# DavidLBick/espnet-1

Hardware: AMD Instinct MI355X
Metric: utterances/sec + step-time, Conformer-L T=1000 batch=32 @1/2/4/8 GPU (higher is better)
Workload: dtype bf16; 1 GPU; C3 Conformer-L (12x512, 8 heads, ff 2048, cnn 31) + 6-layer Transformer decoder, hybrid CTC/att 0.3/0.7, lsm 0.1, V=5000, T=1000 frames x 80, L=40, dropout 0.1, Adam+WarmupLR+clip 5; global_batch=32, seq_len=1000, parallelism=dp1

## Files before the change

espnet-1_amd/csrc/elementwise.hip:

```cpp
#include "common.h"

#include <cstdlib>
#include <cstring>

namespace {

__global__ void mvn_kernel(int B, int T, int F, const float* __restrict__ x, const long long* __restrict__ lens,
                           float* __restrict__ y) {
  const int b = blockIdx.x;
  const int f = threadIdx.x;
  __shared__ double red[1024];
  const long long L = lens[b];
  double s = 0.0;
  const int ty = threadIdx.y, ny = blockDim.y;
  if (f < F)
    for (int t = ty; t < T; t += ny)
      if (t < L) s += x[((long)b * T + t) * F + f];
  red[ty * blockDim.x + f] = s;
  __syncthreads();
  if (ty == 0 && f < F) {
    double a = 0.0;
    for (int k = 0; k < ny; ++k) a += red[k * blockDim.x + f];
    red[f] = a;
  }
// ... 1080 lines not shown
  if (dcol_dtype == EA_BF16 && dtype == EA_BF16) EA_C2I(bf16, bf16);
  else if (dcol_dtype == EA_BF16) EA_C2I(bf16, float);
  else if (dtype == EA_BF16) EA_C2I(float, bf16);
  else EA_C2I(float, float);
#undef EA_C2I
  EA_LAUNCH_CHECK();
  return 0;
}

extern "C" int ea_glu_fwd(long rows, int C, const void* x, int x_dtype, void* y, int y_dtype, void* stream) {
  EA_ENTRY();
  const long n = rows * C;
#define EA_G(TI, TO) hipLaunchKernelGGL((glu_fwd_kernel<TI, TO>), EA_GRID(n), rows, C, (const TI*)x, (TO*)y)
  if (x_dtype == EA_BF16 && y_dtype == EA_BF16) EA_G(bf16, bf16);
  else if (x_dtype == EA_BF16) EA_G(bf16, float);
  else if (y_dtype == EA_BF16) EA_G(float, bf16);
  else EA_G(float, float);
#undef EA_G
  EA_LAUNCH_CHECK();
  return 0;
}

extern "C" int ea_glu_bwd(long rows, int C, const void* x, int x_dtype, const float* dy, void* dx, void* stream) {
  EA_ENTRY();
  const long n = rows * C;
  if (x_dtype == EA_BF16)
    hipLaunchKernelGGL((glu_bwd_kernel<bf16, bf16>), EA_GRID(n), rows, C, (const bf16*)x, dy, (bf16*)dx);
  else
    hipLaunchKernelGGL((glu_bwd_kernel<float, float>), EA_GRID(n), rows, C, (const float*)x, dy, (float*)dx);
  EA_LAUNCH_CHECK();
  return 0;
}

extern "C" int ea_dwconv_fwd(int B, int T, int C, int K, const float* x, const float* w, const float* bias, float* y,
                             void* stream) {
  EA_ENTRY();
  EA_CHECK_ARG(K % 2 == 1);
  dim3 grid(B * ea_cdiv(T, DW_TT), ea_cdiv(C, DW_CT));
  dim3 gridr(B * ea_cdiv(T, 4 * DW_R), ea_cdiv(C, DW_CT));
  hipStream_t st = (hipStream_t)stream;
  switch (K) {
#define EA_DWF(KK) case KK: hipLaunchKernelGGL((dwconv_fwd_k_kernel<KK, DW_R>), gridr, dim3(256), 0, st, B, T, C, x, w, bias, y); break;
    EA_DWF(3) EA_DWF(5) EA_DWF(7) EA_DWF(15) EA_DWF(31)
#undef EA_DWF
    default: {
      const size_t sm = (size_t)(DW_TT + K - 1) * DW_CT * sizeof(float);
      hipLaunchKernelGGL(dwconv_fwd_kernel, grid, dim3(256), sm, st, B, T, C, K, x, w, bias, y);
    }
  }
  EA_LAUNCH_CHECK();
  return 0;
}

extern "C" int ea_dwconv_bwd(int B, int T, int C, int K, const float* x, const float* w, const float* dy, float* dx,
                             float* dw, float* dbias, int accumulate_params, float* workspace, long ws_elems,
                             void* stream) {
  EA_ENTRY();
  EA_CHECK_ARG(K % 2 == 1);
  const int nblk = B * ea_cdiv(T, DW_TT);
  dim3 grid(nblk, ea_cdiv(C, DW_CT));
  if (K == 3 || K == 5 || K == 7 || K == 15 || K == 31) {
    const int nblkr = B * ea_cdiv(T, 4 * DW_R);
    dim3 gridr(nblkr, ea_cdiv(C, DW_CT));
    const long rowlen = (long)C * (K + 1);
    EA_CHECK_ARG((long)nblkr * rowlen <= ws_elems);
    hipStream_t st = (hipStream_t)stream;
    switch (K) {
#define EA_DWB(KK) case KK: hipLaunchKernelGGL((dwconv_bwd_k_kernel<KK, DW_R>), gridr, dim3(256), 0, st, B, T, C, x, w, dy, dx, workspace); break;
      EA_DWB(3) EA_DWB(5) EA_DWB(7) EA_DWB(15) EA_DWB(31)
#undef EA_DWB
    }
    EA_LAUNCH_CHECK();
    int rc = ea_reduce_partials_tr(nblkr, C * K, workspace, rowlen, dw, accumulate_params, C, K, stream);
    if (rc || !dbias) return rc;
    return ea_reduce_partials(nblkr, C, workspace + (long)C * K, rowlen, dbias, accumulate_params, stream);
  }
  EA_CHECK_ARG((long)nblk * C * K <= ws_elems);
  const size_t sm = (size_t)(2 * (DW_TT + K - 1) + DW_TT) * DW_CT * sizeof(float);
  hipStream_t st = (hipStream_t)stream;
  hipLaunchKernelGGL(dwconv_bwd_kernel, grid, dim3(256), sm, st, B, T, C, K, x, w, dy, dx, workspace);
  EA_LAUNCH_CHECK();
  int rc = ea_reduce_partials(nblk, C * K, workspace, (long)C * K, dw, accumulate_params, stream);
  if (rc) return rc;
  if (dbias) return ea_colsum(B * T, C, dy, EA_F32, C, dbias, accumulate_params, workspace, ws_elems, stream);
  return 0;
}

extern "C" int ea_dwconv_fwd_glu(int B, int T, int C, int K, const void* g2, const float* w, const float* bias,
                                 float* y, void* stream) {
  EA_ENTRY();
  EA_CHECK_ARG((K == 3 || K == 5 || K == 7 || K == 15 || K == 31) && g2 && y && C % 4 == 0 &&
               ((uintptr_t)g2 % 8) == 0);
  dim3 gridr(B * ea_cdiv(T, 4 * DW_R), ea_cdiv(C, DW_CT));
  hipStream_t st = (hipStream_t)stream;
  switch (K) {
#define EA_DWF(KK)                                                                                          \
  case KK:                                                                                                  \
    hipLaunchKernelGGL((dwconv_fwd_k_kernel<KK, DW_R, true>), gridr, dim3(256), 0, st, B, T, C, (const float*)nullptr, \
                       w, bias, y, (const bf16*)g2);                                                        \
    break;
    EA_DWF(3) EA_DWF(5) EA_DWF(7) EA_DWF(15) EA_DWF(31)
#undef EA_DWF
  }
  EA_LAUNCH_CHECK();
  return 0;
}

extern "C" int ea_dwconv_fwd_glu_stats(int B, int T, int C, int K, const void* g2, const float* w, const float* bias,
                                       float* y, float* part, void* stream) {
  EA_ENTRY();
  EA_CHECK_ARG((K == 3 || K == 5 || K == 7 || K == 15 || K == 31) && g2 && y && part && bias && C % 4 == 0 &&
               ((uintptr_t)g2 % 8) == 0);
  dim3 gridr(B * ea_cdiv(T, 4 * DW_R), ea_cdiv(C, DW_CT));
  hipStream_t st = (hipStream_t)stream;
  switch (K) {
#define EA_DWF(KK)                                                                                            \
  case KK:                                                                                                    \
    hipLaunchKernelGGL((dwconv_fwd_k_kernel<KK, DW_R, true, true>), gridr, dim3(256), 0, st, B, T, C,           \
                       (const float*)nullptr, w, bias, y, (const bf16*)g2, part);                             \
    break;
    EA_DWF(3) EA_DWF(5) EA_DWF(7) EA_DWF(15) EA_DWF(31)
#undef EA_DWF
  }
  EA_LAUNCH_CHECK();
  return 0;
}

extern "C" int ea_dwconv_stats_parts(int B, int T, int* nparts) {
  EA_ENTRY();
  EA_CHECK_ARG(nparts != nullptr && B > 0 && T > 0);
  *nparts = B * ea_cdiv(T, 4 * DW_R);
  return 0;
}

extern "C" int ea_dwconv_glu_bwd(int B, int T, int C, int K, const float* x, const float* w, const float* dy,
                                 const void* g2, void* dg2, float* dw, float* dbias, int accumulate_params,
                                 float* workspace, long ws_elems, void* stream) {
  EA_ENTRY();
  EA_CHECK_ARG((K == 3 || K == 5 || K == 7 || K == 15 || K == 31) && g2 && dg2 && dw && dbias);
  EA_CHECK_ARG(x != nullptr || (C % 4 == 0 && ((uintptr_t)g2 % 8) == 0));
  const int nblkr = B * ea_cdiv(T, 4 * DW_R);
  dim3 gridr(nblkr, ea_cdiv(C, DW_CT));
  const long rowlen = (long)C * (K + 1);
  EA_CHECK_ARG((long)nblkr * rowlen <= ws_elems);
  hipStream_t st = (hipStream_t)stream;
  const bool adj = dbias == dw + (long)C * K;
  switch (K) {
#define EA_DWB(KK)                                                                                              \
  case KK:                                                                                                      \
    if (x)                                                                                                      \
      hipLaunchKernelGGL((dwconv_bwd_k_kernel<KK, DW_R, false, true>), gridr, dim3(256), 0, st, B, T, C, x, w, dy,   \
                         (float*)nullptr, workspace, (const bf16*)g2, (bf16*)dg2);                                    \
    else                                                                                                        \
      hipLaunchKernelGGL((dwconv_bwd_k_kernel<KK, DW_R, false, true, true>), gridr, dim3(256), 0, st, B, T, C,      \
                         (const float*)nullptr, w, dy, (float*)nullptr, workspace, (const bf16*)g2, (bf16*)dg2);      \
    break;
    EA_DWB(3) EA_DWB(5) EA_DWB(7) EA_DWB(15) EA_DWB(31)
#undef EA_DWB
  }
  EA_LAUNCH_CHECK();
  if (adj) return ea_reduce_partials_tr(nblkr, (int)rowlen, workspace, rowlen, dw, accumulate_params, C, K, stream);
  int rc = ea_reduce_partials_tr(nblkr, C * K, workspace, rowlen, dw, accumulate_params, C, K, stream);
  if (rc) return rc;
  return ea_reduce_partials(nblkr, C, workspace + (long)C * K, rowlen, dbias, accumulate_params, stream);
}


extern "C" int ea_add_pos_bias(long N, int H, int dk, const void* q, long ldq, const float* u, const float* v,
                               void* qu, void* qv, int dtype, void* stream) {
  EA_ENTRY();
  const long n = N * H * dk;
  if (dtype == EA_BF16)
    hipLaunchKernelGGL(add_pos_bias_kernel<bf16>, EA_GRID(n), N, H, dk, (const bf16*)q, ldq, u, v, (bf16*)qu, (bf16*)qv);
  else
    hipLaunchKernelGGL(add_pos_bias_kernel<float>, EA_GRID(n), N, H, dk, (const float*)q, ldq, u, v, (float*)qu, (float*)qv);
  EA_LAUNCH_CHECK();
  return 0;
}

extern "C" int ea_embed_fwd(long rows, int d, int L, const long long* tok, const float* E, float xscale,
                            const float* pe, float p, unsigned long long seed, float* y, void* stream) {
  EA_ENTRY();
  const long n = rows * d;
  hipLaunchKernelGGL(embed_fwd_kernel, EA_GRID(n), rows, d, L, tok, E, xscale, pe, p, (uint64_t)seed, ea_g_rng_salt, y);
  EA_LAUNCH_CHECK();
  return 0;
}

extern "C" int ea_add_pe_dropout(long rows, int d, int L, const float* pe, float p, unsigned long long seed,
                                 float* y, void* stream) {
  EA_ENTRY();
  EA_CHECK_ARG(rows >= 0 && d > 0 && L > 0);
  const long n = rows * d;
  if (n == 0) return 0;
  hipLaunchKernelGGL(add_pe_dropout_kernel, EA_GRID(n), n, d, L, pe, p, (uint64_t)seed, ea_g_rng_salt, y);
  EA_LAUNCH_CHECK();
  return 0;
}

extern "C" int ea_embed_bwd(long rows, int d, const long long* tok, const float* dy, float xscale, float p,
                            unsigned long long seed, float* dE, void* stream) {
  EA_ENTRY();
  EA_CHECK_ARG(rows >= 0 && rows <= EMBED_BWD_MAXROWS);
  if (rows == 0) return 0;
  hipLaunchKernelGGL(embed_bwd_kernel, dim3((unsigned)rows), dim3(256), 0, (hipStream_t)stream, (int)rows, d, tok,
                     dy, xscale, p, (uint64_t)seed, ea_g_rng_salt, dE);
  EA_LAUNCH_CHECK();
  return 0;
}

extern "C" int ea_argmax_rows(long rows, int V, const float* x, long ld, long long* out, void* stream) {
  EA_ENTRY();
  hipLaunchKernelGGL(argmax_rows_kernel, dim3(ea_cdiv(rows, 4)), dim3(256), 0, (hipStream_t)stream, rows, V, x, ld, out);
// ... 111 lines not shown
```

espnet-1_amd/csrc/gemm.hip:

```cpp

#include "gemm_kern.h"
#include <cstdio>
#include <cstdlib>

namespace {
__global__ void splitk_reduce(GemmP p) {
  const long MN = (long)p.M * p.N;
  const int z = blockIdx.y;
  const int zb = z / p.nh, zh = z % p.nh;
  const float* base = p.ws + (long)z * p.splitk * MN;
  const bool vec = p.vec_c && (p.N % 4 == 0);
  const EpiK ek = make_epik(p);
  const long n4 = vec ? MN / 4 : MN;
  for (long i = blockIdx.x * (long)blockDim.x + threadIdx.x; i < n4; i += (long)gridDim.x * blockDim.x) {
    if (vec) {
      float4 a = make_float4(0.f, 0.f, 0.f, 0.f);
      int s = 0;
      for (; s + 8 <= p.splitk; s += 8) {
        float4 b[8];
#pragma unroll
        for (int j = 0; j < 8; ++j) b[j] = *(const float4*)(base + (long)(s + j) * MN + i * 4);
#pragma unroll
        for (int j = 0; j < 8; ++j) { a.x += b[j].x; a.y += b[j].y; a.z += b[j].z; a.w += b[j].w; }
      }
      for (; s < p.splitk; ++s) {
        const float4 b = *(const float4*)(base + (long)s * MN + i * 4);
        a.x += b.x; a.y += b.y; a.z += b.z; a.w += b.w;
      }
      const int row = (int)(i * 4 / p.N), col = (int)(i * 4 % p.N);
      const float v[4] = {a.x, a.y, a.z, a.w};
      switch (p.epi.kind) {
        case EA_EPI_STORE: epi_four<EA_EPI_STORE>(p, ek, z, zb, zh, row, col, v); break;
        case EA_EPI_ACT: epi_four<EA_EPI_ACT>(p, ek, z, zb, zh, row, col, v); break;
        case EA_EPI_RESID: epi_four<EA_EPI_RESID>(p, ek, z, zb, zh, row, col, v); break;
        default: epi_four<EA_EPI_DACT>(p, ek, z, zb, zh, row, col, v); break;
      }
    } else {
      float a = 0.f;
      for (int s = 0; s < p.splitk; ++s) a += base[s * MN + i];
      epi_apply(p, z, zb, zh, (int)(i / p.N), (int)(i % p.N), a);
    }
  }
}

int g_gemm_stages = 2;
unsigned long long* g_probe = nullptr;
unsigned long long* g_diag = nullptr;
int g_gemm_bm64 = 1;
int g_gemm_bm32 = [] { const char* e = std::getenv("EA_GEMM_BM32"); return e ? std::atoi(e) : 1; }();
int g_gemm_pipe = 0;

int g_gemm_k128 = [] { const char* e = std::getenv("EA_GEMM_K128"); return e ? std::atoi(e) : 1; }();
int g_gemm_skinny = [] { const char* e = std::getenv("EA_GEMM_SKINNY"); return e ? std::atoi(e) : 16; }();

int launch_lds(GemmP& p, int a_k, int b_k, int nz, hipStream_t st, bool k128 = false) {
  dim3 grid(p.tiles_m * p.tiles_n, 1, nz * p.splitk);
  if (k128) return launch_k128(p, grid, st);
  if (p.g.mode != 0) {
    if (p.bm == 256 && g_gemm_pipe) return launch_pipe_conv(p, grid, st);
    return launch_lds_conv(p, grid, st);
  }
  if ((p.bm == 256 && p.bn == 256 && (g_gemm_pipe & 1)) ||
      (p.bm == 128 && p.bn == 128 && (g_gemm_pipe & 2)))
    return launch_pipe(p, a_k, b_k, grid, st);
  return launch_lds_dense(p, a_k, b_k, grid, st);
}

int g_force_bm = 0, g_force_bn = 0;
void choose_tile(GemmP& p, int a_k, long nz) {
  struct Cfg { int bm, bn, occ; double t0, rcu; bool ak_only; };
  static const Cfg cfgs[] = {{256, 256, 1, 12.4, 4.49, false}, {128, 128, 2, 8.3, 2.9, false},
                             {64, 128, 3, 6.8, 2.8, true}, {32, 128, 2, 6.0, 2.0, true}};
  p.bm = 128; p.bn = 128;
  if (g_force_bm) {
    if (g_force_bm <= 64 && !a_k) return;
    p.bm = g_force_bm; p.bn = g_force_bn;
    return;
  }
  double best = 1e300;
  for (const Cfg& c : cfgs) {
    if (c.ak_only && (!a_k || !g_gemm_bm64)) continue;
    if (c.bm == 32 && !g_gemm_bm32) continue;
    const long tiles = (long)ea_cdiv(p.M, c.bm) * ea_cdiv(p.N, c.bn) * nz;
    const double rounds = (double)((tiles + 256L * c.occ - 1) / (256L * c.occ));
    const double per_cu = (double)((tiles + 255) / 256) * 2.0 * c.bm * c.bn * (double)p.K * 1e-6;
    const double est = rounds * c.t0 + per_cu / c.rcu;
    if (est < best * 0.999) { best = est; p.bm = c.bm; p.bn = c.bn; }
  }
}

template <typename T>
int launch(GemmP& p, int a_k, int b_k, int nz, hipStream_t st, bool k128 = false) {
  if (sizeof(T) == 2 && p.lds) return launch_lds(p, a_k, b_k, nz, st, k128);
  if (p.bm != 128 || p.bn != 128) return EA_ERR_BAD_ARG;
  dim3 grid(p.tiles_m * p.tiles_n, 1, nz * p.splitk);
#define EA_GEMM_CASE(AKV, BKV)                                                      \
  if (a_k == AKV && b_k == BKV) {                                                   \
    hipLaunchKernelGGL((gemm_kernel<T, AKV, BKV>), grid, dim3(NT), 0, st, p);       \
  }
  EA_GEMM_CASE(true, true)
  else EA_GEMM_CASE(true, false)
  else EA_GEMM_CASE(false, true)
  else EA_GEMM_CASE(false, false)
#undef EA_GEMM_CASE
  EA_LAUNCH_CHECK();
  return 0;
}

}

extern "C" int ea_gemm_set_pipeline(int stages) {
  EA_ENTRY();
  EA_CHECK_ARG(stages == 0 || stages == 2 || stages == 12);
  g_gemm_bm64 = stages < 10;
  g_gemm_stages = stages % 10;
  return 0;
}

namespace {
__global__ void probe_begin_kernel(unsigned long long* s) { s[0] = ~0ull; s[1] = 0ull; }
__global__ void probe_end_kernel(unsigned long long* s) {
// ... 35 lines not shown
  EA_CHECK_ARG(state != nullptr && ring != nullptr && cap > 0 && phase >= 0 && phase <= 3 && opt != nullptr);
  hipLaunchKernelGGL(phase_stamp_kernel, dim3(1), dim3(1), 0, (hipStream_t)stream, state, ring, cap, phase,
                     &opt->next_lr, &opt->skip);
  EA_LAUNCH_CHECK();
  return 0;
}

extern "C" int ea_gemm_set_diag(unsigned long long* buf) {
  EA_ENTRY();
  g_diag = buf;
  return 0;
}

extern "C" int ea_gemm_set_probe(unsigned long long* slots) {
  EA_ENTRY();
  g_probe = slots;
  return 0;
}

extern "C" int ea_probe_begin(unsigned long long* slots, void* stream) {
  EA_ENTRY();
  EA_CHECK_ARG(slots != nullptr);
  hipLaunchKernelGGL(probe_begin_kernel, dim3(1), dim3(1), 0, (hipStream_t)stream, slots);
  EA_LAUNCH_CHECK();
  return 0;
}

extern "C" int ea_probe_end(unsigned long long* slots, void* stream) {
  EA_ENTRY();
  EA_CHECK_ARG(slots != nullptr);
  hipLaunchKernelGGL(probe_end_kernel, dim3(1), dim3(1), 0, (hipStream_t)stream, slots);
  EA_LAUNCH_CHECK();
  return 0;
}

extern "C" int ea_gemm_set_pipe(int on) {
  EA_ENTRY();
  g_gemm_pipe = on;
  return 0;
}

extern "C" int ea_gemm_set_k128(int mode, int slots) {
  EA_ENTRY();
  EA_CHECK_ARG(mode >= 0 && mode <= 3 && (slots == 3 || slots == 4));
  g_gemm_k128 = mode;
  eag::g_k128_slots = slots;
  return 0;
}

extern "C" int ea_gemm_set_skinny(int max_m) {
  EA_ENTRY();
  EA_CHECK_ARG(max_m >= 0 && max_m <= 64);
  g_gemm_skinny = max_m;
  return 0;
}

extern "C" int ea_gemm_set_tile(int bm, int bn) {
  EA_ENTRY();
  EA_CHECK_ARG((bm == 0 && bn == 0) || (bm == 32 && bn == 128) || (bm == 64 && bn == 128) ||
               (bm == 128 && bn == 128) || (bm == 256 && bn == 256));
  g_force_bm = bm;
  g_force_bn = bn;
  return 0;
}

static int gemm_impl(int dtype, int a_kmajor, int b_kmajor, int M, int N, int K,
                     const void* A, long lda, long sAb, long sAh,
                     const void* B, long ldb, long sBb, long sBh,
                     int batch, int nh,
                     void* C, int c_dtype, long ldc, long sCb, long sCh,
                     const ea_epilogue* epi, float* workspace, long ws_elems, void* stream,
                     const ea_conv_geo* geo, const float* w1x = nullptr, int w1T = 0, int w1F = 0,
                     float* w1part = nullptr, const uint8_t* w1pos = nullptr) {
  EA_CHECK_ARG(epi != nullptr && M >= 0 && N >= 0 && K >= 0 && batch >= 1 && nh >= 1);
  EA_CHECK_ARG(dtype == EA_F32 || dtype == EA_BF16);
  if (M == 0 || N == 0) return 0;
  const int E = dtype == EA_BF16 ? 8 : 4;
  const int esz = dtype == EA_BF16 ? 2 : 4;
  (void)esz;
  if (epi->kind == EA_EPI_RESID) EA_CHECK_ARG(c_dtype == EA_F32);
  GemmP p{};
  p.M = M; p.N = N; p.K = K;
  p.A = A; p.lda = lda; p.sAb = sAb; p.sAh = sAh;
  p.B = B; p.ldb = ldb; p.sBb = sBb; p.sBh = sBh;
  p.nh = nh;
  p.C = C; p.c_dtype = c_dtype; p.ldc = ldc; p.sCb = sCb; p.sCh = sCh;
  p.epi = *epi;
  p.ws = workspace;
  p.salt = ea_g_rng_salt;
  p.stamp = g_probe;
  p.diag = g_diag;
  p.g = geo ? *geo : ea_conv_geo{};
  p.w1x = w1x; p.w1part = w1part; p.w1pos = w1pos; p.w1T = w1T; p.w1F = w1F;
  p.vec_a = (lda % E == 0 && sAb % E == 0 && sAh % E == 0 && ((uintptr_t)A % 16) == 0);
  p.vec_b = (ldb % E == 0 && sBb % E == 0 && sBh % E == 0 && ((uintptr_t)B % 16) == 0);
  {
    const int ce = c_dtype == EA_BF16 ? 2 : 4;
    bool vc = (N % 4 == 0) && ldc % 4 == 0 && sCb % 4 == 0 && sCh % 4 == 0 && ((uintptr_t)C % (4 * ce)) == 0;
    if (epi->bias) vc = vc && ((uintptr_t)epi->bias % 16) == 0;
    if (epi->aux) vc = vc && epi->ldaux % 4 == 0 && ((uintptr_t)epi->aux % (4 * (epi->aux_dtype == EA_BF16 ? 2 : 4))) == 0;
    if (epi->resid) vc = vc && epi->ldr % 4 == 0 && ((uintptr_t)epi->resid % 16) == 0;
    p.vec_c = vc;
    bool v8 = vc && N % 8 == 0 && ldc % 8 == 0 && sCb % 8 == 0 && sCh % 8 == 0 && ((uintptr_t)C % 16) == 0;
    if (epi->aux) v8 = v8 && epi->ldaux % 8 == 0 && ((uintptr_t)epi->aux % 16) == 0;
    if (epi->resid) v8 = v8 && epi->ldr % 8 == 0;
    p.vec8 = v8;
  }
  p.bm = 128; p.bn = 128;
  if (dtype == EA_BF16 && M <= g_gemm_skinny && a_kmajor && b_kmajor && !geo && !w1part &&
      batch * nh == 1 && K % 32 == 0 && K > 0 && p.vec_a && p.vec_b) {
    static const bool trace_s = std::getenv("EA_GEMM_TRACE") != nullptr;
    if (trace_s) std::fprintf(stderr, "[ea_gemm] M=%d N=%d K=%d skinny epi=%d\n", M, N, K, (int)epi->kind);
    return launch_skinny(p, (hipStream_t)stream);
  }
  const double a_ext = 2.0 * ((a_kmajor ? (double)M : (double)K) * lda);
  const double b_ext = 2.0 * ((b_kmajor ? (double)N : (double)K) * ldb);
  const bool lds_path = dtype == EA_BF16 && p.vec_a && p.vec_b && g_gemm_stages > 0 &&
                        a_ext < 4.0e9 && b_ext < 4.0e9;
  p.lds = lds_path;
  if (geo && geo->mode != 0) {
    if (!lds_path || K % 64 != 0 || geo->C % 64 != 0 || batch * nh != 1) return EA_ERR_BAD_ARG;
    if ((geo->mode == EA_CONV_WGRAD) == (a_kmajor != 0) || (geo->mode == EA_CONV_FWD) != (b_kmajor != 0))
      return EA_ERR_BAD_ARG;
    choose_tile(p, 0, 1);
    if (geo->mode == EA_CONV_WGRAD && !g_force_bm) { p.bm = 256; p.bn = 256; }
    if (w1part) {
      if (!g_gemm_pipe || !p.vec8) return EA_ERR_BAD_ARG;
      p.bm = 256; p.bn = 256;
    }
    if (p.bm != 256 || p.bn != 256) { p.bm = 128; p.bn = 128; }
  } else if (lds_path) {
    choose_tile(p, a_kmajor, (long)batch * nh);
  }
  bool k128 = false;
  if (g_gemm_k128 && lds_path && !geo && a_kmajor && b_kmajor && K % 64 == 0 && K > 0) {
    const long t128 = (long)ea_cdiv(M, 128) * ea_cdiv(N, 128) * batch * nh;
    const bool fits = g_gemm_k128 == 3 ||
                      (!g_force_bm && (p.bm == 64 || p.bm == 128) && p.bn == 128 && t128 >= 128 &&
                       (g_gemm_k128 == 2 || (t128 <= 256 && K >= 1024)));
    if (fits) { p.bm = 128; p.bn = 128; k128 = true; }
  }
  if (p.bm <= 64 && !a_kmajor) return EA_ERR_BAD_ARG;
  p.tiles_m = ea_cdiv(M, p.bm);
  p.tiles_n = ea_cdiv(N, p.bn);
  const int KT = dtype == EA_BF16 ? KCfg<bf16>::KT : KCfg<float>::KT;
  const int nz = batch * nh;
  int splitk = 1;
  const long tiles = max(1L, (long)p.tiles_m * p.tiles_n * nz * (p.bm * p.bn) / (128 * 128));
  if (geo && geo->mode == EA_CONV_WGRAD && p.bm == 256) {
    if (workspace) {
      splitk = max(1, 256 / (p.tiles_m * p.tiles_n));
      splitk = min(splitk, K / (4 * KT));
      while (splitk > 1 && (long)splitk * M * N > ws_elems) --splitk;
      splitk = max(splitk, 1);
    }
  } else if (!k128 && workspace && tiles < 200 && K >= 16 * KT && K >= 1024 && (long)p.tiles_m * p.tiles_n * nz < 128) {
    splitk = (int)((384 + tiles - 1) / tiles);
    splitk = min(splitk, K / (4 * KT));
    splitk = min(splitk, 16);
    while (splitk > 1 && (long)splitk * nz * M * N > ws_elems) --splitk;
    if (splitk < 1) splitk = 1;
  }
  int kchunk = K;
  if (splitk > 1) {
    kchunk = ea_cdiv(ea_cdiv(K, splitk), KT) * KT;
    splitk = ea_cdiv(K, kchunk);
  }
  p.splitk = splitk;
  p.kchunk = kchunk;
  static const bool trace = std::getenv("EA_GEMM_TRACE") != nullptr;
  if (trace)
    std::fprintf(stderr, "[ea_gemm] M=%d N=%d K=%d ak=%d bk=%d nz=%d tile=%dx%d%s splitk=%d epi=%d geo=%d lds=%d\n", M,
                 N, K, a_kmajor, b_kmajor, nz, p.bm, p.bn, k128 ? "k" : "", splitk, (int)epi->kind, geo ? geo->mode : 0,
                 (int)p.lds);
  hipStream_t st = (hipStream_t)stream;
  int rc = dtype == EA_BF16 ? launch<bf16>(p, a_kmajor, b_kmajor, nz, st, k128)
                            : launch<float>(p, a_kmajor, b_kmajor, nz, st);
  if (rc) return rc;
  if (splitk > 1) {
    const long MN = (long)M * N;
    dim3 grid(ea_grid_cap(ea_cdiv(MN / 4 + 1, 256), 2048), nz);
    hipLaunchKernelGGL(splitk_reduce, grid, dim3(256), 0, st, p);
    EA_LAUNCH_CHECK();
  }
  return 0;
}

extern "C" int ea_gemm(int dtype, int a_kmajor, int b_kmajor, int M, int N, int K,
                       const void* A, long lda, long sAb, long sAh,
                       const void* B, long ldb, long sBb, long sBh,
                       int batch, int nh,
                       void* C, int c_dtype, long ldc, long sCb, long sCh,
                       const ea_epilogue* epi, float* workspace, long ws_elems, void* stream) {
  EA_ENTRY();
  return gemm_impl(dtype, a_kmajor, b_kmajor, M, N, K, A, lda, sAb, sAh, B, ldb, sBb, sBh, batch, nh, C, c_dtype,
                   ldc, sCb, sCh, epi, workspace, ws_elems, stream, nullptr);
}

extern "C" int ea_gemm_ln(int M, int N, int K, const float* x, long ldx, const float* gamma, const float* beta,
                          float eps, const void* W, long ldw, void* C, int c_dtype, long ldc, const ea_epilogue* epi,
                          void* stream) {
  EA_ENTRY();
  EA_CHECK_ARG(epi != nullptr && M >= 0 && N >= 0 && K > 0 && K % 32 == 0 && K <= 32 * 8 * 8);
  EA_CHECK_ARG(x && gamma && beta && W && C && ldx >= K && ldw >= K && ldc >= N);
  EA_CHECK_ARG(ldx % 4 == 0 && ((uintptr_t)x % 16) == 0 && ldw % 8 == 0 && ((uintptr_t)W % 16) == 0 &&
               ((uintptr_t)gamma % 16) == 0 && ((uintptr_t)beta % 16) == 0);
  if (epi->kind == EA_EPI_RESID) EA_CHECK_ARG(c_dtype == EA_F32);
  if (M == 0 || N == 0) return 0;
  GemmP p{};
  p.M = M; p.N = N; p.K = K;
  p.A = x; p.lda = ldx;
  p.B = W; p.ldb = ldw;
  p.nh = 1; p.splitk = 1; p.kchunk = K;
  p.C = C; p.c_dtype = c_dtype; p.ldc = ldc;
  p.epi = *epi;
  p.salt = ea_g_rng_salt;
  const int ce = c_dtype == EA_BF16 ? 2 : 4;
  bool vc = (N % 4 == 0) && ldc % 4 == 0 && ((uintptr_t)C % (4 * ce)) == 0;
  if (epi->bias) vc = vc && ((uintptr_t)epi->bias % 16) == 0;
  if (epi->aux) vc = vc && epi->ldaux % 4 == 0 && ((uintptr_t)epi->aux % (4 * (epi->aux_dtype == EA_BF16 ? 2 : 4))) == 0;
  if (epi->resid) vc = vc && epi->ldr % 4 == 0 && ((uintptr_t)epi->resid % 16) == 0;
  p.vec_c = vc;
  return launch_skinny_ln(p, gamma, beta, eps, (hipStream_t)stream);
}

extern "C" int ea_gemm_conv(const ea_conv_geo* geo, int a_kmajor, int b_kmajor, int M, int N, int K,
                            const void* A, long lda, const void* B, long ldb, void* C, int c_dtype, long ldc,
                            const ea_epilogue* epi, float* workspace, long ws_elems, void* stream) {
  EA_ENTRY();
  EA_CHECK_ARG(geo != nullptr && geo->mode >= EA_CONV_FWD && geo->mode <= EA_CONV_WGRAD);
  return gemm_impl(EA_BF16, a_kmajor, b_kmajor, M, N, K, A, lda, 0, 0, B, ldb, 0, 0, 1, 1, C, c_dtype, ldc, 0, 0,
                   epi, workspace, ws_elems, stream, geo);
}

extern "C" int ea_gemm_conv_w1(const ea_conv_geo* geo, int M, int N, int K, const void* A, long lda, const void* B,
                               long ldb, const ea_epilogue* epi, const float* x, int T, int Fin, float* part,
                               void* stream) {
  EA_ENTRY();
  EA_CHECK_ARG(geo != nullptr && geo->mode == EA_CONV_DGRAD && x != nullptr && part != nullptr);
  EA_CHECK_ARG(epi != nullptr && epi->kind == EA_EPI_DACT && epi->act == EA_ACT_RELU && epi->aux != nullptr &&
               epi->aux_dtype == EA_BF16);
  EA_CHECK_ARG(T >= 3 && Fin >= 3 && M < (1 << 24));
  return gemm_impl(EA_BF16, 1, 0, M, N, K, A, lda, 0, 0, B, ldb, 0, 0, 1, 1, nullptr, EA_BF16, N, 0, 0, epi,
                   nullptr, 0, stream, geo, x, T, Fin, part);
}

extern "C" int ea_gemm_conv_w1b(const ea_conv_geo* geo, int M, int N, int K, const void* A, long lda, const void* B,
                                long ldb, const ea_epilogue* epi, const float* x, int T, int Fin, float* part,
                                const unsigned char* pos, void* stream) {
  EA_ENTRY();
  EA_CHECK_ARG(geo != nullptr && geo->mode == EA_CONV_DGRAD && x != nullptr && part != nullptr && pos != nullptr);
  EA_CHECK_ARG(epi != nullptr && epi->kind == EA_EPI_DACT && epi->act == EA_ACT_RELU && N % 8 == 0);
  EA_CHECK_ARG(T >= 3 && Fin >= 3 && M < (1 << 24));
  return gemm_impl(EA_BF16, 1, 0, M, N, K, A, lda, 0, 0, B, ldb, 0, 0, 1, 1, nullptr, EA_BF16, N, 0, 0, epi,
                   nullptr, 0, stream, geo, x, T, Fin, part, pos);
}


extern "C" int ea_gemm_conv_w1b_all(const ea_conv_geo* geo, int N, const void* A, long lda, const void* B, long ldb,
                                    const ea_epilogue* epi, const float* x, int T, int Fin, float* part,
                                    const unsigned char* pos, void* stream) {
  EA_ENTRY();
  EA_CHECK_ARG(geo != nullptr && geo->mode == EA_CONV_DGRAD && x != nullptr && part != nullptr && pos != nullptr);
  EA_CHECK_ARG(epi != nullptr && epi->kind == EA_EPI_DACT && epi->act == EA_ACT_RELU);
  EA_CHECK_ARG(N >= 8 && N % 8 == 0 && geo->C % 64 == 0 && T >= 3 && Fin >= 3 && g_gemm_pipe != 0);
  EA_CHECK_ARG(lda % 8 == 0 && ldb % 8 == 0 && ((uintptr_t)A % 16) == 0 && ((uintptr_t)B % 16) == 0);
  GemmP p{};
  p.N = N;
  p.A = A; p.lda = lda;
  p.B = B; p.ldb = ldb;
  p.nh = 1; p.splitk = 1;
  p.C = nullptr; p.c_dtype = EA_BF16; p.ldc = N;
  p.epi = *epi;
  p.salt = ea_g_rng_salt;
  p.stamp = g_probe;
  p.diag = g_diag;
  p.g = *geo;
  p.w1x = x; p.w1part = part; p.w1pos = pos; p.w1T = T; p.w1F = Fin;
  p.vec_a = p.vec_b = p.vec_c = p.vec8 = p.lds = 1;
  p.bm = p.bn = 256;
  p.tiles_n = ea_cdiv(N, 256);
  int items = 0, tiles = 0;
  for (int c = 0; c < 4; ++c) {
    const int a = c >> 1, e = c & 1;
    const long rows = (long)geo->B * geo->nI[a] * geo->nJ[e];
    EA_CHECK_ARG(rows < (1L << 24));
    if (rows == 0) continue;
    const int k = p.ncls++;
    p.cls_item0[k] = items;
    p.cls_M[k] = (int)rows;
    p.cls_K[k] = (a ? 1 : 2) * (e ? 1 : 2) * geo->C;
    p.cls_a[k] = a;
    p.cls_e[k] = e;
    p.cls_tile0[k] = tiles;
    p.cls_pos[k] = geo->plane[c] / geo->C * (N / 8);
    tiles += (int)ea_cdiv(rows, 256);
    items += (int)ea_cdiv(rows, 256) * p.tiles_n;
  }
  if (p.ncls == 0) return 0;
  p.cls_item0[p.ncls] = items;
  p.M = p.cls_M[0]; p.K = p.cls_K[0]; p.kchunk = p.K; p.tiles_m = ea_cdiv(p.M, 256);
  const int unit = 8 * p.tiles_n;
  const dim3 grid((unsigned)(ea_cdiv(items, unit) * unit));
  static const bool trace = std::getenv("EA_GEMM_TRACE") != nullptr;
  if (trace) std::fprintf(stderr, "[ea_gemm] conv dgrad x%d classes, %d tiles, grid %u\n", p.ncls, items, grid.x);
  return launch_pipe_conv(p, grid, (hipStream_t)stream);
}
```

espnet-1_amd/csrc/gemm_kern.h:

```cpp
#pragma once
#include "common.h"


namespace eag {

constexpr int BM = 128, BN = 128, NT = 256;
constexpr int TILE_BYTES = 16384;

template <typename T> struct KCfg;
template <> struct KCfg<bf16> { static constexpr int KT = 64, KS = 32, E = 8, NKS = 2; };
template <> struct KCfg<float> { static constexpr int KT = 32, KS = 4, E = 4, NKS = 8; };

struct GemmP {
  int M, N, K;
  const void* A; long lda, sAb, sAh;
  const void* B; long ldb, sBb, sBh;
  int nh, splitk, kchunk;
  void* C; int c_dtype; long ldc, sCb, sCh;
  ea_epilogue epi;
  float* ws;
  int tiles_m, tiles_n;
  int vec_a, vec_b;
  int vec_c;
  int vec8;
// ... 256 lines not shown
    if (has_o) {
#pragma unroll
      for (int c = 0; c < 4; ++c) v[c] += e.beta * o[c];
    }
    st4(p.C, cidx, p.c_dtype, v);
  } else if constexpr (KIND == EA_EPI_ACT) {
    if (e.aux) st4(e.aux, (long)row * e.ldaux + col, e.aux_dtype, v);
    act_fwd_n<4>(e.act, v);
    drop4k(k, didx, v);
    st4(p.C, cidx, p.c_dtype, v);
  } else if constexpr (KIND == EA_EPI_RESID) {
    drop4k(k, didx, v);
#pragma unroll
    for (int c = 0; c < 4; ++c) v[c] = (has_o ? o[c] : 0.f) + e.rscale * v[c];
    st4(p.C, cidx, EA_F32, v);
  } else {
    drop4k(k, didx, v);
    act_bwd_mul_n<4>(e.act, v, o);
    st4(p.C, cidx, p.c_dtype, v);
  }
}

EA_DEV void ld8(const void* p, long i, int dt, float (&v)[8]) {
  if (dt == EA_BF16) {
    const uint4 u = *(const uint4*)((const bf16*)p + i);
    const bf16* b = (const bf16*)&u;
#pragma unroll
    for (int c = 0; c < 8; ++c) v[c] = (float)b[c];
  } else {
    const float4 f0 = *(const float4*)((const float*)p + i), f1 = *(const float4*)((const float*)p + i + 4);
    v[0] = f0.x; v[1] = f0.y; v[2] = f0.z; v[3] = f0.w; v[4] = f1.x; v[5] = f1.y; v[6] = f1.z; v[7] = f1.w;
  }
}
EA_DEV void st8(void* p, long i, int dt, const float (&v)[8]) {
  if (dt == EA_BF16) {
    union { uint4 u; bf16 b[8]; } t;
#pragma unroll
    for (int c = 0; c < 8; ++c) t.b[c] = (bf16)v[c];
    *(uint4*)((bf16*)p + i) = t.u;
  } else {
    *(float4*)((float*)p + i) = make_float4(v[0], v[1], v[2], v[3]);
    *(float4*)((float*)p + i + 4) = make_float4(v[4], v[5], v[6], v[7]);
  }
}
EA_DEV void drop8k(const EpiK& k, uint64_t idx, float (&v)[8]) {
  if (!k.drop) return;
#pragma unroll
  for (int q = 0; q < 4; ++q) {
    const uint32_t h = ea_pair_hash(k.key, (idx >> 1) + q);
    v[2 * q] *= (h & 0xffffu) >= k.thr ? k.sc : 0.f;
    v[2 * q + 1] *= (h >> 16) >= k.thr ? k.sc : 0.f;
  }
}
template <int KIND>
EA_DEV void epi_eight_pre(const GemmP& p, const EpiK& k, int z, int zb, int zh, int row, int col,
                          const float (&acc)[8], const float (&bias)[8], bool has_o, const float (&o)[8]) {
  const ea_epilogue& e = p.epi;
  const long cidx = zb * p.sCb + zh * p.sCh + (long)row * p.ldc + col;
  const uint64_t didx = ((uint64_t)z * p.M + row) * (uint64_t)p.N + col;
  float v[8];
#pragma unroll
  for (int c = 0; c < 8; ++c) v[c] = e.alpha * acc[c] + (KIND != EA_EPI_DACT ? bias[c] : 0.f);
  if constexpr (KIND == EA_EPI_STORE) {
#pragma unroll
    for (int c = 0; c < 8; ++c) v[c] *= e.post_scale;
    drop8k(k, didx, v);
    if (has_o) {
#pragma unroll
      for (int c = 0; c < 8; ++c) v[c] += e.beta * o[c];
    }
    st8(p.C, cidx, p.c_dtype, v);
  } else if constexpr (KIND == EA_EPI_ACT) {
    if (e.aux) st8(e.aux, (long)row * e.ldaux + col, e.aux_dtype, v);
    act_fwd_n<8>(e.act, v);
    drop8k(k, didx, v);
    st8(p.C, cidx, p.c_dtype, v);
  } else if constexpr (KIND == EA_EPI_RESID) {
    drop8k(k, didx, v);
#pragma unroll
    for (int c = 0; c < 8; ++c) v[c] = (has_o ? o[c] : 0.f) + e.rscale * v[c];
    st8(p.C, cidx, EA_F32, v);
  } else {
    drop8k(k, didx, v);
    act_bwd_mul_n<8>(e.act, v, o);
    st8(p.C, cidx, p.c_dtype, v);
  }
}

template <int KIND>
EA_DEV void epi_four(const GemmP& p, const EpiK& k, int z, int zb, int zh, int row, int col, const float (&acc)[4]) {
  float bias[4] = {0.f, 0.f, 0.f, 0.f}, o[4];
  if (p.epi.bias) {
    const float4 bb = *(const float4*)(p.epi.bias + col);
    bias[0] = bb.x; bias[1] = bb.y; bias[2] = bb.z; bias[3] = bb.w;
  }
  const bool has_o = epi_src<KIND>(p, zb, zh, row, col, o);
  epi_four_pre<KIND>(p, k, z, zb, zh, row, col, acc, bias, has_o, o);
}

template <int KIND, int NB>
EA_DEV void epi_batch(const GemmP& p, const EpiK& k, int z, int zb, int zh, const int (&rows)[NB],
                      const int (&cols)[NB], const float (&v)[NB][4]) {
  float o[NB][4];
  bool has[NB];
#pragma unroll
  for (int i = 0; i < NB; ++i) {
    has[i] = false;
    if (rows[i] < p.M && cols[i] < p.N) has[i] = epi_src<KIND>(p, zb, zh, rows[i], cols[i], o[i]);
  }
#pragma unroll
  for (int i = 0; i < NB; ++i) {
    if (rows[i] >= p.M || cols[i] >= p.N) continue;
    float bias[4] = {0.f, 0.f, 0.f, 0.f};
    if (KIND != EA_EPI_DACT && p.epi.bias) {
      const float4 bb = *(const float4*)(p.epi.bias + cols[i]);
      bias[0] = bb.x; bias[1] = bb.y; bias[2] = bb.z; bias[3] = bb.w;
    }
    epi_four_pre<KIND>(p, k, z, zb, zh, rows[i], cols[i], v[i], bias, has[i], o[i]);
  }
}

constexpr int EPI_LDT = 68;

template <typename T, bool AK, bool BKM>
__global__ __launch_bounds__(NT, 2) void gemm_kernel(GemmP p) {
  constexpr int KT = KCfg<T>::KT, NKS = KCfg<T>::NKS;
  __shared__ __attribute__((aligned(16))) char smem[2][2][TILE_BYTES];

  const int nt = p.tiles_m * p.tiles_n;
  const int b = blockIdx.x;
  const int q = nt / 8, r = nt % 8, xcd = b % 8;
  const int t = (xcd < r ? xcd * (q + 1) : r * (q + 1) + (xcd - r) * q) + b / 8;
  const int GM = 8;
  const int grp = t / (GM * p.tiles_n);
  const int gm0 = grp * GM;
  const int gsz = min(GM, p.tiles_m - gm0);
  const int tm = gm0 + (t % (GM * p.tiles_n)) % gsz;
  const int tn = (t % (GM * p.tiles_n)) / gsz;
// ... 126 lines not shown
                        uint4 (&v)[ROWS * 8 / NTT]) {
  constexpr int NCH = ROWS * 8 / NTT;
#pragma unroll
  for (int i = 0; i < NCH; ++i) {
    const int c = threadIdx.x + NTT * i;
    int mn, k;
    if (KMAJ) { mn = mn0 + (c >> 3); k = k0 + (c & 7) * 8; }
    else      { const int cj = c & 1023; k = k0 + (cj >> 4); mn = mn0 + (c >> 10) * 128 + (cj & 15) * 8; }
    const bf16* pp = KMAJ ? base + (long)mn * ld + k : base + (long)k * ld + mn;
    union { uint4 u; bf16 e[8]; } t;
#pragma unroll
    for (int e = 0; e < 8; ++e) {
      const bool ok = KMAJ ? (mn < MN && k + e < K) : (k < K && mn + e < MN);
      t.e[e] = ok ? pp[e] : (bf16)0.f;
    }
    v[i] = t.u;
  }
}
template <bool KMAJ, int ROWS, int NTT>
EA_DEV void store_tile_r(char* lds, const uint4 (&v)[ROWS * 8 / NTT]) {
#pragma unroll
  for (int i = 0; i < ROWS * 8 / NTT; ++i) {
    const int c = threadIdx.x + NTT * i;
    *(uint4*)(lds + img_off<KMAJ>(c)) = v[i];
  }
}

template <bool KMAJ>
EA_DEV bf16x8 frag_img(const char* img, int r, int ks, int lane) {
  if (KMAJ) return frag_bf16<true>(img, r, ks, lane);
  return frag_bf16<false>(img + (r >> 7) * 16384, r & 127, ks, lane);
}

struct TileIdx { int tm, tn, z, sk; };
EA_DEV TileIdx tile_index(const GemmP& p) {
  const int nt = p.tiles_m * p.tiles_n;
  const int total = gridDim.x * gridDim.z;
  const int bid = blockIdx.x + gridDim.x * blockIdx.z;
  const int q = total / 8, r = total % 8, xcd = bid % 8;
  const int w = (xcd < r ? xcd * (q + 1) : r * (q + 1) + (xcd - r) * q) + bid / 8;
  const int zz = w / nt, t = w - zz * nt;
  const int GM = 8;
  const int grp = t / (GM * p.tiles_n);
  const int gm0 = grp * GM;
  const int gsz = min(GM, p.tiles_m - gm0);
  TileIdx ti;
  ti.tm = gm0 + (t % (GM * p.tiles_n)) % gsz;
  ti.tn = (t % (GM * p.tiles_n)) / gsz;
  ti.z = zz / p.splitk;
  ti.sk = zz % p.splitk;
  return ti;
}

template <int KIND, int MI, int NJ>
EA_DEV void epi_wave(const GemmP& p, const EpiK& k, char* smem, int z, int zb, int zh, int r0, int c0, int lane,
                     int w, const f32x4 (&acc)[MI][NJ], int sk = 0) {
  constexpr int RC = MI < 4 ? MI : 4;
  constexpr int NG = RC * 4;
  constexpr int HB = NG < 8 ? NG : 8;
  constexpr int NCH = (MI / RC) * (NJ / 4), NBC = NG / HB, NU = NCH * NBC;
  float* t = (float*)smem + w * (RC * 16) * EPI_LDT;
  const int rq = (lane >> 4) * 4, cc = lane & 15, lc = (lane & 15) * 4;
  float* slab = p.splitk > 1 ? p.ws + ((long)z * p.splitk + sk) * (long)p.M * p.N : nullptr;
  const bool reads = p.vec_c && !slab &&
                     (KIND == EA_EPI_DACT || (KIND == EA_EPI_RESID && p.epi.resid) ||
                      (KIND == EA_EPI_STORE && p.epi.beta != 0.f));
  const void* src = nullptr;
  long sld = 0, sbase = 0;
  int sdt = EA_F32;
  if constexpr (KIND == EA_EPI_STORE) {
    src = p.C; sld = p.ldc; sbase = zb * p.sCb + zh * p.sCh; sdt = p.c_dtype;
  } else if constexpr (KIND == EA_EPI_RESID) {
    src = p.epi.resid; sld = p.epi.ldr;
  } else if constexpr (KIND == EA_EPI_DACT) {
    src = p.epi.aux; sld = p.epi.ldaux; sdt = p.epi.aux_dtype;
  }
  auto ch_rb = [&](int ch) { return r0 + (ch / (NJ / 4)) * RC * 16; };
  auto ch_col = [&](int ch) { return c0 + (ch % (NJ / 4)) * 64 + lc; };
  auto load_unit = [&](int u, float (&o)[HB][4]) {
    if (!reads) return;
    const int ch = u / NBC, h0 = (u % NBC) * HB;
    const int rb = ch_rb(ch), cl = min(ch_col(ch), p.N - 4);
    if (sdt == EA_BF16) {
#pragma unroll
      for (int it = 0; it < HB; ++it)
        vld4((const bf16*)src + sbase + (long)min(rb + (h0 + it) * 4 + (lane >> 4), p.M - 1) * sld + cl, o[it]);
    } else {
#pragma unroll
      for (int it = 0; it < HB; ++it)
        vld4((const float*)src + sbase + (long)min(rb + (h0 + it) * 4 + (lane >> 4), p.M - 1) * sld + cl, o[it]);
    }
  };
  auto transpose = [&](int ch) {
    const int ri = ch / (NJ / 4), cj = ch % (NJ / 4);
    if (ch > 0) {
      __builtin_amdgcn_wave_barrier();
      asm volatile("" ::: "memory");
    }
#pragma unroll
    for (int i = 0; i < RC; ++i)
#pragma unroll
      for (int j = 0; j < 4; ++j)
#pragma unroll
        for (int rr = 0; rr < 4; ++rr)
          t[(i * 16 + rq + rr) * EPI_LDT + j * 16 + cc] = acc[ri * RC + i][cj * 4 + j][rr];
    __builtin_amdgcn_wave_barrier();
    asm volatile("" ::: "memory");
  };
  if (!p.vec_c) {
#pragma unroll
    for (int ch = 0; ch < NCH; ++ch) {
      transpose(ch);
      const int rb = ch_rb(ch), col = ch_col(ch);
#pragma unroll 1
      for (int it = 0; it < NG; ++it) {
        const int lr = it * 4 + (lane >> 4), row = rb + lr;
        if (row >= p.M) continue;
#pragma unroll 1
        for (int c = 0; c < 4; ++c) {
          if (col + c >= p.N) break;
          const float x = t[lr * EPI_LDT + lc + c];
          if (slab) slab[(long)row * p.N + col + c] = x;
          else epi_one<KIND>(p, z, zb, zh, row, col + c, x);
        }
      }
    }
    return;
  }
  if (p.vec8) {
    constexpr int NG8 = RC * 2;
    constexpr int HB8 = NG8 < 4 ? NG8 : 4;
    const int lc8 = (lane & 7) * 8, rl = lane >> 3;
#pragma unroll
    for (int ch = 0; ch < NCH; ++ch) {
      transpose(ch);
      const int rb = ch_rb(ch), col = c0 + (ch % (NJ / 4)) * 64 + lc8;
      float bias[8] = {0.f, 0.f, 0.f, 0.f, 0.f, 0.f, 0.f, 0.f};
      if (!slab && KIND != EA_EPI_DACT && p.epi.bias && col < p.N) {
        const float4 b0 = *(const float4*)(p.epi.bias + col), b1 = *(const float4*)(p.epi.bias + col + 4);
        bias[0] = b0.x; bias[1] = b0.y; bias[2] = b0.z; bias[3] = b0.w;
        bias[4] = b1.x; bias[5] = b1.y; bias[6] = b1.z; bias[7] = b1.w;
      }
#pragma unroll
      for (int h0 = 0; h0 < NG8; h0 += HB8) {
        float o[HB8][8];
        if (reads) {
          const int cl = min(col, p.N - 8);
          if (sdt == EA_BF16) {
#pragma unroll
            for (int it = 0; it < HB8; ++it)
              ld8(src, sbase + (long)min(rb + (h0 + it) * 8 + rl, p.M - 1) * sld + cl, EA_BF16, o[it]);
          } else {
#pragma unroll
            for (int it = 0; it < HB8; ++it)
              ld8(src, sbase + (long)min(rb + (h0 + it) * 8 + rl, p.M - 1) * sld + cl, EA_F32, o[it]);
          }
        }
#pragma unroll
        for (int it = 0; it < HB8; ++it) {
          const int lr = (h0 + it) * 8 + rl, row = rb + lr;
          const float4 f0 = *(const float4*)(t + lr * EPI_LDT + lc8), f1 = *(const float4*)(t + lr * EPI_LDT + lc8 + 4);
          if (row >= p.M || col >= p.N) continue;
          if (slab) {
            *(float4*)(slab + (long)row * p.N + col) = f0;
            *(float4*)(slab + (long)row * p.N + col + 4) = f1;
            continue;
          }
          const float v[8] = {f0.x, f0.y, f0.z, f0.w, f1.x, f1.y, f1.z, f1.w};
          epi_eight_pre<KIND>(p, k, z, zb, zh, row, col, v, bias, reads, o[it]);
        }
      }
    }
    return;
  }
#pragma unroll
  for (int u = 0; u < NU; ++u) {
    const int ch = u / NBC, h0 = (u % NBC) * HB;
    const int rb = ch_rb(ch), col = ch_col(ch);
    if (u % NBC == 0) transpose(ch);
    float ob[HB][4];
    load_unit(u, ob);
    float bias[4] = {0.f, 0.f, 0.f, 0.f};
    if (!slab && KIND != EA_EPI_DACT && p.epi.bias && col < p.N) {
      const float4 bb = *(const float4*)(p.epi.bias + col);
      bias[0] = bb.x; bias[1] = bb.y; bias[2] = bb.z; bias[3] = bb.w;
    }
#pragma unroll
    for (int it = 0; it < HB; ++it) {
      const int lr = (h0 + it) * 4 + (lane >> 4), row = rb + lr;
      const float4 f = *(const float4*)(t + lr * EPI_LDT + lc);
      if (row >= p.M || col >= p.N) continue;
      const float v[4] = {f.x, f.y, f.z, f.w};
      if (slab) *(float4*)(slab + (long)row * p.N + col) = f;
      else epi_four_pre<KIND>(p, k, z, zb, zh, row, col, v, bias, reads, ob[it]);
    }
  }
}

EA_DEV int fdiv(int n, int d) {
  int q = (int)((float)n * __builtin_amdgcn_rcpf((float)d));
  if (q * d > n) --q;
  if ((q + 1) * d <= n) ++q;
  return q;
}
EA_DEV long x1p_row(const ea_conv_geo& g, int b, int t2, int f2, int kh, int kw) {
  const int a = kh & 1, e = kw & 1;
  return g.plane[a * 2 + e] + (((long)b * g.nI[a] + t2 + (kh >> 1)) * g.nJ[e] + f2 + (kw >> 1)) * g.C;
}
EA_DEV void dgrad_tap2(int a, int e, int q, int& kh, int& kw) {
  const int nkw = e ? 1 : 2;
  const int qh = q / nkw, qw = q - qh * nkw;
  kh = a ? 1 : 2 * qh;
  kw = e ? 1 : 2 * qw;
}
EA_DEV void dgrad_tap(const ea_conv_geo& g, int q, int& kh, int& kw) {
  const int nkw = g.e ? 1 : 2;
  const int qh = q / nkw, qw = q - qh * nkw;
  kh = g.a ? 1 : 2 * qh;
  kw = g.e ? 1 : 2 * qw;
}

template <int BM_, int BN_, int WN, bool AK, bool BKM, int STAGES, int MODE = 0>
// ... 176 lines not shown
          acc[i][j] = __builtin_amdgcn_mfma_f32_16x16x32_bf16(fa0[i], fb0[j], acc[i][j], 0, 0, 0);
#pragma unroll
      for (int i = 0; i < MI; ++i)
#pragma unroll
        for (int j = 0; j < NJ; ++j)
          acc[i][j] = __builtin_amdgcn_mfma_f32_16x16x32_bf16(fa1[i], fb1[j], acc[i][j], 0, 0, 0);
    } else {
#pragma unroll
      for (int ks = 0; ks < 2; ++ks) {
        bf16x8 fb[NJ];
#pragma unroll
        for (int j = 0; j < NJ; ++j) fb[j] = frag_img<BKM>(lb, wn + j * 16, ks, lane);
#pragma unroll
        for (int i = 0; i < MI; ++i) {
          const bf16x8 fa = frag_img<AK>(la, wm + i * 16, ks, lane);
#pragma unroll
          for (int j = 0; j < NJ; ++j)
            acc[i][j] = __builtin_amdgcn_mfma_f32_16x16x32_bf16(fa, fb[j], acc[i][j], 0, 0, 0);
        }
      }
    }
  };

  const int npre = min(STAGES - 1, nfull);
  for (int kt = 0; kt < npre; ++kt) issue(kt, kt);
  for (int kt = 0; kt < nfull; ++kt) {
    const int after = min(STAGES - 2, nfull - 1 - kt);
    if (after >= 2) wait_vmcnt<2 * GPT>();
    else if (after == 1) wait_vmcnt<GPT>();
    else wait_vmcnt<0>();
    lds_barrier();
    if (kt + STAGES - 1 < nfull) issue(kt + STAGES - 1, (kt + STAGES - 1) % STAGES);
    compute(kt % STAGES);
  }
  if (tail) {
    uint4 ra[BM_ * 8 / NTT], rb[BN_ * 8 / NTT];
    const int k0 = kbeg + nfull * BK;
    load_tile_r<AK, BM_, NTT>(A, p.lda, m0, p.M, k0, kend, ra);
    load_tile_r<BKM, BN_, NTT>(B, p.ldb, n0, p.N, k0, kend, rb);
    __syncthreads();
    char* base = smem + (nfull % STAGES) * STAGE_BYTES;
    store_tile_r<AK, BM_, NTT>(base, ra);
    store_tile_r<BKM, BN_, NTT>(base + A_BYTES, rb);
    __syncthreads();
    compute(nfull % STAGES);
  }

  __syncthreads();
  const EpiK ek = make_epik(p);
  switch (p.splitk > 1 ? EA_EPI_STORE : p.epi.kind) {
    case EA_EPI_STORE: epi_wave<EA_EPI_STORE, MI, NJ>(p, ek, smem, z, zb, zh, m0 + wm, n0 + wn, lane, w, acc, sk); break;
    case EA_EPI_ACT: epi_wave<EA_EPI_ACT, MI, NJ>(p, ek, smem, z, zb, zh, m0 + wm, n0 + wn, lane, w, acc, sk); break;
    case EA_EPI_RESID: epi_wave<EA_EPI_RESID, MI, NJ>(p, ek, smem, z, zb, zh, m0 + wm, n0 + wn, lane, w, acc, sk); break;
    default: epi_wave<EA_EPI_DACT, MI, NJ>(p, ek, smem, z, zb, zh, m0 + wm, n0 + wn, lane, w, acc, sk); break;
  }
  probe_end(p);
}

template <int OFF>
EA_DEV bf16x8 ds_read_b128_at(uint32_t addr) {
  bf16x8 v;
  asm volatile("ds_read_b128 %0, %1 offset:%2" : "=v"(v) : "v"(addr), "i"(OFF) : "memory");
  return v;
}

template <int S>
__global__ __launch_bounds__(512, 1) void gemm_k128(GemmP p) {
  constexpr int BK = 64, NTT = 512, NW = 8, MI = 4, NJ = 4;
  constexpr int A_BYTES = 128 * BK * 2, B_BYTES = 128 * BK * 2, STAGE = A_BYTES + B_BYTES;
  constexpr int ACH = A_BYTES / (NTT * 16), BCH = B_BYTES / (NTT * 16), G = ACH + BCH;
  constexpr int EPI_BYTES = 4 * 4 * 16 * EPI_LDT * 4;
  constexpr int HAND = EPI_BYTES;
  constexpr int SMEM = S * STAGE > HAND + 65536 ? S * STAGE : HAND + 65536;
  static_assert(S >= 3 && S <= 4, "ring depth");
  __shared__ __attribute__((aligned(1024))) char smem[SMEM];
  probe_start(p);

  const TileIdx ti = tile_index(p);
  const int m0 = ti.tm * 128, n0 = ti.tn * 128;
  const int z = ti.z, sk = ti.sk;
  const int zb = z / p.nh, zh = z % p.nh;
  const bf16* A = (const bf16*)p.A + zb * p.sAb + zh * p.sAh;
  const bf16* B = (const bf16*)p.B + zb * p.sBb + zh * p.sBh;
  const int kbeg = sk * p.kchunk;
  const int kend = min(p.K, kbeg + p.kchunk);
  const int nt = max(0, (kend - kbeg) / BK);
  const int tid = threadIdx.x, lane = tid & 63;
  const int w = __builtin_amdgcn_readfirstlane(tid >> 6);
  const int g = w >> 2, q = w & 3;
  const int wm = (q >> 1) * 64, wn = (q & 1) * 64;

  const __amdgpu_buffer_rsrc_t ra = __builtin_amdgcn_make_buffer_rsrc(
      (void*)(A + kbeg), (short)0, 0x7fffffff, 0x00020000);
  const __amdgpu_buffer_rsrc_t rb = __builtin_amdgcn_make_buffer_rsrc(
      (void*)(B + kbeg), (short)0, 0x7fffffff, 0x00020000);
  auto src = [&](long ld, int mn0, int MN, int ci) -> uint32_t {
    const int row = ci >> 3, c = (ci & 7) ^ swz_k(ci >> 3);
    return (uint32_t)(((long)min(mn0 + row, MN - 1) * ld + c * 8) * 2);
  };
  uint32_t aoff[ACH], boff[BCH];
#pragma unroll
  for (int i = 0; i < ACH; ++i) aoff[i] = src(p.lda, m0, p.M, (i * NW + w) * 64 + lane);
#pragma unroll
  for (int i = 0; i < BCH; ++i) boff[i] = src(p.ldb, n0, p.N, (i * NW + w) * 64 + lane);

  auto issue = [&](int t) {
    char* base = smem + (t % S) * STAGE;
// ... 529 lines not shown
  for (int k = 1; k < 4; ++k) c += (k < p.ncls && item >= p.cls_item0[k]) ? 1 : 0;
  const int local = item - p.cls_item0[c];
  ov.M = p.cls_M[c];
  ov.a = p.cls_a[c];
  ov.e = p.cls_e[c];
  ov.w1part = p.w1part + (long)p.cls_tile0[c] * 10 * p.N;
  ov.w1pos = p.w1pos + p.cls_pos[c];
  ti.tm = local / tn_n;
  ti.tn = local % tn_n;
  ti.z = 0;
  ti.sk = p.cls_K[c];
  return true;
}

template <bool AK, bool BKM, int MODE, int BT, int NS>
EA_DEV void pipe_body(const GemmP& p, const TileOv& ov, const TileIdx& ti, char* smem) {
  using PC = PipeT<BT, NS>;
  constexpr int MI = PC::MI;
  const int tm = ti.tm, m0 = ti.tm * BT, n0 = ti.tn * BT;
  const bool cls = MODE == EA_CONV_DGRAD && p.ncls;
  const int z = ti.z, sk = cls ? 0 : ti.sk;
  const int zb = z / p.nh, zh = z % p.nh;
  const bf16* A = (const bf16*)p.A + zb * p.sAb + zh * p.sAh;
  const bf16* B = (const bf16*)p.B + zb * p.sBb + zh * p.sBh;
  const int kbeg = sk * p.kchunk;
  const int kend = cls ? ti.sk : min(p.K, kbeg + p.kchunk);
  const int tid = threadIdx.x, lane = tid & 63, w = tid >> 6;
  const int wm = PC::wm(w), wn = PC::wn(w);
  f32x4 acc[MI][4];
#pragma unroll
  for (int i = 0; i < MI; ++i)
#pragma unroll
    for (int j = 0; j < 4; ++j) acc[i][j] = (f32x4){0.f, 0.f, 0.f, 0.f};
  diag_stamp(p, 0);
  float w1x[5];
  if constexpr (MODE == EA_CONV_DGRAD) {
    if (p.w1part) w1_load_x(p, ov, m0, w1x);
  }
  pipe_tile<AK, BKM, MODE, BT, NS>(p, ov, smem, A, B, m0, n0, kbeg, kend, acc);
  diag_stamp(p, 1);
  if constexpr (MODE == EA_CONV_DGRAD) {
    if (p.w1part) {
      w1_stage_x(smem + PC::SMEM, w1x);
      __syncthreads();
      w1_epilogue(p, ov, smem, m0, n0, wm, wn, lane, w, tm, acc);
      return;
    }
  }
  const EpiK ek = make_epik(p);
  switch (p.splitk > 1 ? EA_EPI_STORE : p.epi.kind) {
    case EA_EPI_STORE: epi_wave<EA_EPI_STORE, MI, 4>(p, ek, smem, z, zb, zh, m0 + wm, n0 + wn, lane, w, acc, sk); break;
    case EA_EPI_ACT: epi_wave<EA_EPI_ACT, MI, 4>(p, ek, smem, z, zb, zh, m0 + wm, n0 + wn, lane, w, acc, sk); break;
    case EA_EPI_RESID: epi_wave<EA_EPI_RESID, MI, 4>(p, ek, smem, z, zb, zh, m0 + wm, n0 + wn, lane, w, acc, sk); break;
    default: epi_wave<EA_EPI_DACT, MI, 4>(p, ek, smem, z, zb, zh, m0 + wm, n0 + wn, lane, w, acc, sk); break;
  }
  if (p.diag) {
    __syncthreads();
    diag_stamp(p, 2);
  }
}

template <bool AK, bool BKM, int MODE = 0, int BT = 256, int NS = 4>
__global__ __launch_bounds__(512, (PipeT<BT, NS>::OCC)) void gemm_pipe(GemmP p) {
  using PC = PipeT<BT, NS>;
  __shared__ __attribute__((aligned(1024))) char smem[MODE == EA_CONV_DGRAD ? W1_SMEM : PC::SMEM];
  probe_start(p);
  TileOv ov = tile_ov(p);
  TileIdx ti;
  bool run = true;
  if (MODE == EA_CONV_DGRAD && p.ncls) run = dgrad_class_item(p, ov, ti);
  else ti = tile_index(p);
  if (run) pipe_body<AK, BKM, MODE, BT, NS>(p, ov, ti, smem);
  probe_end(p);
}

}
```

espnet-1_amd/csrc/reduce.hip:

```cpp
#include "common.h"

namespace {

struct ColsumProbD {
  const void* x;
  float* part;
  long ld;
  int rows, n, dtype, rpp, ncb, item0;
};

struct ReduceProbD {
  const float* part;
  float* out;
  long stride;
  int nparts, n, accumulate, item0;
};

constexpr int CHUNK = 40;
template <typename P>
struct Chunk {
  int first, n;
  P pr[CHUNK];
};
static_assert(sizeof(Chunk<ColsumProbD>) <= 4000 && sizeof(Chunk<ReduceProbD>) <= 4000, "kernel argument space");

template <typename P>
__global__ void table_upload(Chunk<P> c, P* table) {
  for (int i = threadIdx.x; i < c.n; i += blockDim.x) table[c.first + i] = c.pr[i];
}

template <typename P>
EA_DEV int find_prob(const P* table, int n, int t) {
  int lo = 0, hi = n - 1;
  while (lo < hi) {
    const int mid = (lo + hi + 1) >> 1;
    if (__builtin_amdgcn_readfirstlane(table[mid].item0) <= t) lo = mid;
    else hi = mid - 1;
  }
  return lo;
}

__global__ __launch_bounds__(256) void colsum_grouped_kernel(const ColsumProbD* __restrict__ table, int nprob) {
  __shared__ float red[4][256];
  const int pi = find_prob(table, nprob, blockIdx.x);
  const ColsumProbD q = table[pi];
  const int it = blockIdx.x - q.item0;
  const int rb = it / q.ncb, cb = it - rb * q.ncb;
  const int lane = threadIdx.x & 63, w = threadIdx.x >> 6;
  const int c = cb * 256 + lane * 4;
  const int r0 = rb * q.rpp, r1 = min(q.rows, r0 + q.rpp);
  float a[4] = {0.f, 0.f, 0.f, 0.f};
  if (c < q.n) {
    if (q.dtype == EA_BF16) {
      const bf16* x = (const bf16*)q.x;
      int r = r0 + w;
      for (; r + 12 < r1; r += 16) {
        float v[4][4];
#pragma unroll
        for (int j = 0; j < 4; ++j) vld4(x + (long)(r + 4 * j) * q.ld + c, v[j]);
#pragma unroll
        for (int j = 0; j < 4; ++j)
#pragma unroll
          for (int k = 0; k < 4; ++k) a[k] += v[j][k];
      }
      for (; r < r1; r += 4) {
        float v[4];
        vld4(x + (long)r * q.ld + c, v);
#pragma unroll
        for (int k = 0; k < 4; ++k) a[k] += v[k];
      }
    } else {
      const float* x = (const float*)q.x;
      int r = r0 + w;
      for (; r + 12 < r1; r += 16) {
        float v[4][4];
#pragma unroll
        for (int j = 0; j < 4; ++j) vld4(x + (long)(r + 4 * j) * q.ld + c, v[j]);
#pragma unroll
        for (int j = 0; j < 4; ++j)
#pragma unroll
          for (int k = 0; k < 4; ++k) a[k] += v[j][k];
      }
      for (; r < r1; r += 4) {
        float v[4];
        vld4(x + (long)r * q.ld + c, v);
#pragma unroll
        for (int k = 0; k < 4; ++k) a[k] += v[k];
      }
    }
  }
#pragma unroll
  for (int k = 0; k < 4; ++k) red[w][lane * 4 + k] = a[k];
  __syncthreads();
  const int cc = cb * 256 + threadIdx.x;
  const int t = threadIdx.x;
  if (cc < q.n) q.part[(long)rb * q.n + cc] = (red[0][t] + red[1][t]) + (red[2][t] + red[3][t]);
}

constexpr int RP_CW = 16, RP_PL = 16;
__global__ __launch_bounds__(256) void reduce_grouped_kernel(const ReduceProbD* __restrict__ table, int nprob) {
  __shared__ double red[RP_PL][RP_CW];
  const int pi = find_prob(table, nprob, blockIdx.x);
  const ReduceProbD q = table[pi];
  const int cx = threadIdx.x % RP_CW, py = threadIdx.x / RP_CW;
  const int c = (blockIdx.x - q.item0) * RP_CW + cx;
  double a = 0.0;
  if (c < q.n) {
    int p = py;
    for (; p + 7 * RP_PL < q.nparts; p += 8 * RP_PL) {
      float v[8];
#pragma unroll
      for (int j = 0; j < 8; ++j) v[j] = q.part[(long)(p + RP_PL * j) * q.stride + c];
#pragma unroll
      for (int j = 0; j < 8; ++j) a += v[j];
    }
    for (; p < q.nparts; p += RP_PL) a += q.part[(long)p * q.stride + c];
  }
  red[py][cx] = a;
  __syncthreads();
  if (py == 0 && c < q.n) {
    double t = 0.0;
#pragma unroll
    for (int l = 0; l < RP_PL; ++l) t += red[l][cx];
    q.out[c] = q.accumulate ? q.out[c] + (float)t : (float)t;
  }
}

template <typename P>
int upload(const P* probs, int n, P* table, hipStream_t st) {
  Chunk<P> c{};
  for (int i = 0; i < n; ++i) {
    c.pr[c.n++] = probs[i];
    if (c.n == CHUNK || i == n - 1) {
      hipLaunchKernelGGL((table_upload<P>), dim3(1), dim3(64), 0, st, c, table);
      EA_LAUNCH_CHECK();
      c.first += c.n;
      c.n = 0;
    }
  }
  return 0;
}

}

extern "C" int ea_colsum_grouped(int n, const ea_colsum_prob* probs, void* ws, long ws_bytes, void* stream) {
  EA_ENTRY();
  EA_CHECK_ARG(n >= 0 && (n == 0 || (probs && ws)));
  if (n == 0) return 0;
  EA_CHECK_ARG((long)n * (long)sizeof(ColsumProbD) <= ws_bytes && n <= 4096);
  ColsumProbD* host = (ColsumProbD*)malloc(sizeof(ColsumProbD) * n);
  if (!host) return EA_ERR_BAD_ARG;
  long items = 0;
  int rc = 0;
  for (int i = 0; i < n && !rc; ++i) {
    const ea_colsum_prob& e = probs[i];
    const bool ok = e.x && e.part && e.rows > 0 && e.n > 0 && e.n % 4 == 0 && e.ld % 4 == 0 && e.rpp > 0 &&
                    (e.dtype == EA_BF16 || e.dtype == EA_F32) &&
                    ((uintptr_t)e.x % (e.dtype == EA_BF16 ? 8 : 16)) == 0;
    if (!ok) { rc = EA_ERR_BAD_ARG; break; }
    ColsumProbD& d = host[i];
    d.x = e.x; d.part = e.part; d.ld = e.ld;
    d.rows = e.rows; d.n = e.n; d.dtype = e.dtype; d.rpp = e.rpp;
    d.ncb = ea_cdiv(e.n, 256);
    d.item0 = (int)items;
    items += (long)ea_cdiv(e.rows, e.rpp) * d.ncb;
  }
  if (!rc && items >= (1L << 30)) rc = EA_ERR_BAD_ARG;
  hipStream_t st = (hipStream_t)stream;
  if (!rc) rc = upload(host, n, (ColsumProbD*)ws, st);
  free(host);
  if (rc) return rc;
  hipLaunchKernelGGL(colsum_grouped_kernel, dim3((unsigned)items), dim3(256), 0, st, (const ColsumProbD*)ws, n);
  EA_LAUNCH_CHECK();
  return 0;
}

extern "C" int ea_reduce_grouped(int n, const ea_reduce_prob* probs, void* ws, long ws_bytes, void* stream) {
  EA_ENTRY();
  EA_CHECK_ARG(n >= 0 && (n == 0 || (probs && ws)));
  if (n == 0) return 0;
  EA_CHECK_ARG((long)n * (long)sizeof(ReduceProbD) <= ws_bytes && n <= 4096);
  ReduceProbD* host = (ReduceProbD*)malloc(sizeof(ReduceProbD) * n);
  if (!host) return EA_ERR_BAD_ARG;
  long items = 0;
  int rc = 0;
  for (int i = 0; i < n; ++i) {
    const ea_reduce_prob& e = probs[i];
    if (!(e.part && e.out && e.n > 0 && e.nparts >= 0 && e.stride >= e.n)) { rc = EA_ERR_BAD_ARG; break; }
    ReduceProbD& d = host[i];
    d.part = e.part; d.out = e.out; d.stride = e.stride;
    d.nparts = e.nparts; d.n = e.n; d.accumulate = e.accumulate;
    d.item0 = (int)items;
    items += ea_cdiv(e.n, RP_CW);
  }
  if (!rc && items >= (1L << 30)) rc = EA_ERR_BAD_ARG;
  hipStream_t st = (hipStream_t)stream;
  if (!rc) rc = upload(host, n, (ReduceProbD*)ws, st);
  free(host);
  if (rc) return rc;
  hipLaunchKernelGGL(reduce_grouped_kernel, dim3((unsigned)items), dim3(256), 0, st, (const ReduceProbD*)ws, n);
  EA_LAUNCH_CHECK();
  return 0;
}

extern "C" int ea_grouped_table_bytes(int n, long* colsum_bytes, long* reduce_bytes) {
  EA_CHECK_ARG(n >= 0 && colsum_bytes && reduce_bytes);
  *colsum_bytes = (long)n * (long)sizeof(ColsumProbD);
  *reduce_bytes = (long)n * (long)sizeof(ReduceProbD);
  return 0;
}
```

espnet-1_amd/espnet_amd/deferred.py:

```python
from __future__ import annotations

import contextlib
import ctypes
import os

import torch

from ._lib import ColsumProb, GroupGemm, ReduceProb, dt, lib
from .streams import WGRAD, on_side, scratch, stream

GRAD_READY = None

DEFER_WGRAD = os.environ.get("EA_DEFER_WGRAD", "1") != "0"
DEFER_BUDGET = int(float(os.environ.get("EA_DEFER_BUDGET_MB", "8192")) * 2 ** 20)


def _nbytes(t):
    return t.numel() * t.element_size()


class WgradQueue:

    def __init__(self):
        self.active = False
# ... 47 lines not shown
                t.record_stream(cur)
        arr = (GroupGemm * n)()
        ntiles = 0
        for i, (K, dy, x, dw, M, N, lda, ldb, ldc, beta, _, _) in enumerate(items):
            arr[i] = GroupGemm(dy.data_ptr(), x.data_ptr(), dw.data_ptr(), lda, ldb, ldc, M, N, K, beta)
            ntiles += ((M + 255) // 256) * ((N + 255) // 256)
        nbytes = ctypes.c_long(0)
        lib.ea_gemm_grouped_ws_bytes(n, ntiles, ctypes.addressof(nbytes))
        ws = scratch("ggemm", nbytes.value, items[0][1].device)
        lib.ea_gemm_grouped(0, 0, n, ctypes.addressof(arr), ws.data_ptr(), ws.numel(), stream())
        for post in posts:
            post()

    def tensors(self):
        return [t for it in self.items for t in (it[1], it[2])]


WGRAD_Q = WgradQueue()

DEFER_REDUCE = os.environ.get("EA_DEFER_REDUCE", "1") != "0"


class ReduceQueue:

    def __init__(self):
        self.active = False
        self.colsums = []
        self.reduces = []
        self.spans = []
        self.pending = 0

    def _account(self, t):
        self.pending += _nbytes(t)
        if self.pending > DEFER_BUDGET:
            self.flush()

    def _claim(self, out, n):
        lo = out.data_ptr()
        hi = lo + 4 * n
        if any(lo < h and l_ < hi for l_, h in self.spans):
            self.flush()
        self.spans.append((lo, hi))

    def add_colsum(self, x, rows, n, ld, out, accumulate) -> bool:
        if x.dtype not in (torch.bfloat16, torch.float32) or out.dtype != torch.float32 or not out.is_contiguous():
            return False
        if rows <= 0 or n % 4 or ld % 4 or x.data_ptr() % (8 if x.dtype == torch.bfloat16 else 16):
            return False
        self._claim(out, n)
        self.colsums.append((x, rows, n, ld, out, accumulate))
        self._account(x)
        return True

    def add_reduce(self, part, nparts, n, stride, out, accumulate=True):
        self._claim(out, n)
        self.reduces.append((part, nparts, n, stride, out, accumulate))
        self._account(part)

    def tensors(self):
        return [c[0] for c in self.colsums] + [r[0] for r in self.reduces]

    def flush(self):
        if not self.colsums and not self.reduces:
            return
        colsums, reduces = self.colsums, list(self.reduces)
        self.colsums, self.reduces, self.spans = [], [], []
        self.pending = 0
        cur = torch.cuda.current_stream()
        for t in [c[0] for c in colsums] + [r[0] for r in reduces]:
            t.record_stream(cur)
        dev = (colsums[0][0] if colsums else reduces[0][0]).device
        cb, rb = ctypes.c_long(0), ctypes.c_long(0)
        if colsums:
            rpps = [max(32, (c[1] + 127) // 128) for c in colsums]
            nrbs = [(c[1] + r - 1) // r for c, r in zip(colsums, rpps)]
            part = torch.empty(sum(nrb * c[2] for c, nrb in zip(colsums, nrbs)), dtype=torch.float32, device=dev)
            arr = (ColsumProb * len(colsums))()
            off = 0
            for i, ((x, rows, n, ld, out, acc), rpp, nrb) in enumerate(zip(colsums, rpps, nrbs)):
                arr[i] = ColsumProb(x.data_ptr(), part.data_ptr() + 4 * off, ld, rows, n, dt(x), rpp)
                reduces.append((part, nrb, n, n, out, acc, off))
                off += nrb * n
            lib.ea_grouped_table_bytes(len(colsums), ctypes.addressof(cb), ctypes.addressof(rb))
            ws = scratch("colsum", cb.value, dev)
            lib.ea_colsum_grouped(len(colsums), ctypes.addressof(arr), ws.data_ptr(), ws.numel(), stream())
        arr = (ReduceProb * len(reduces))()
        for i, r in enumerate(reduces):
            part, nparts, n, stride, out, acc = r[:6]
            off = r[6] if len(r) > 6 else 0
            arr[i] = ReduceProb(part.data_ptr() + 4 * off, out.data_ptr(), stride, nparts, n, int(acc))
        lib.ea_grouped_table_bytes(len(reduces), ctypes.addressof(cb), ctypes.addressof(rb))
        ws = scratch("reduce", rb.value, dev)
        lib.ea_reduce_grouped(len(reduces), ctypes.addressof(arr), ws.data_ptr(), ws.numel(), stream())


REDUCE_Q = ReduceQueue()


def wgrad(*tensors, after=None, launches=False):
    if not launches and WGRAD_Q.active and REDUCE_Q.active:
        return contextlib.nullcontext()
    return WGRAD(*tensors, after=after)


def fork_event():
    return None if GRAD_READY is not None else WGRAD.fork_point()


def join_wgrad():
    WGRAD.join()
    WGRAD_Q.side_events = []


def grad_ready(bound):
    if GRAD_READY is not None:
        GRAD_READY(bound.prefix)
        return
    join_wgrad()


def _side_flush_ok():
    return GRAD_READY is None and WGRAD.enabled and torch.cuda.is_available()


def flush_wgrad_side(after=None):
    if WGRAD_Q.active and WGRAD_Q.items and _side_flush_ok():
        with WGRAD(*WGRAD_Q.tensors(), after=after):
            WGRAD_Q.flush()


def flush_deferred():
    WGRAD_Q.flush()
    REDUCE_Q.flush()


def deferred_tensors():
    return WGRAD_Q.tensors() + REDUCE_Q.tensors()


class deferred_wgrad:

    def __enter__(self):
        self.prev = (WGRAD_Q.active, REDUCE_Q.active)
# ... 20 lines not shown
```

espnet-1_amd/espnet_amd/hip_ops.py:

```python
from __future__ import annotations

import ctypes
import os
import sys
import types
import weakref

import torch

from . import deferred, streams
from ._lib import ACT_NONE, EPI_STORE, Epilogue, HipError, dt, lib
from .deferred import (REDUCE_Q, WGRAD_Q, deferred_tensors, deferred_wgrad, flush_deferred,
                       flush_wgrad_side, fork_event, grad_ready, join_wgrad, wgrad)
from .streams import aux, join_aux, mark_aux_fork, on_side, scratch, stream, take_aux_fork

_MOVED = {**dict.fromkeys(("DEBUG_DELAY_NS", "DEBUG_SERIAL", "OVERLAP_CTC_BWD"), streams),
          **dict.fromkeys(("GRAD_READY", "DEFER_WGRAD", "DEFER_REDUCE", "DEFER_BUDGET"), deferred)}


class _Ops(types.ModuleType):
    def __getattr__(self, name):
        if name in _MOVED:
            return getattr(_MOVED[name], name)
        raise AttributeError(f"module {self.__name__!r} has no attribute {name!r}")

    def __setattr__(self, name, value):
        if name in _MOVED:
            setattr(_MOVED[name], name, value)
        else:
            super().__setattr__(name, value)


sys.modules[__name__].__class__ = _Ops


class KernelProbe:

    TICK_MS = 1e-5

    def __init__(self, names, device=None):
        self.names = set(names)
        dev = device or torch.device("cuda", torch.cuda.current_device())
        self.slots = {n: torch.zeros(4, dtype=torch.int64, device=dev) for n in names}
        self.active = True

    def begin(self, name):
        if self.active and name in self.names:
            s = self.slots[name].data_ptr()
            lib.ea_probe_begin(s, stream())
            lib.ea_gemm_set_probe(s)

    def end(self, name):
        if self.active and name in self.names:
            lib.ea_gemm_set_probe(None)
            lib.ea_probe_end(self.slots[name].data_ptr(), stream())

    def reset(self):
        for t in self.slots.values():
            t.zero_()

    def mean_ms(self, name):
        tot, cnt = (int(x) for x in self.slots[name][2:4].tolist())
        return (tot / cnt * self.TICK_MS if cnt else float("nan")), cnt

# ... 146 lines not shown
        self.frozen = False

    def _rebuild(self):
        probs, tiles = [], []
        for pi, ((off, R, C), dst) in enumerate(self.items.items()):
            probs.append((off, dst.data_ptr(), R | (C << 32)))
            tiles += [(pi, tr, tc, 0) for tr in range((R + 63) // 64) for tc in range((C + 63) // 64)]
        dev = self.shadow.device
        self.probs = torch.tensor(probs, dtype=torch.int64).to(dev)
        self.tiles = torch.tensor(tiles, dtype=torch.int32).to(dev)
        self.ntiles = len(tiles)

    def get(self, w):
        off = (w.data_ptr() - self.shadow.data_ptr()) // w.element_size()
        key = (off, int(w.shape[0]), int(w.shape[1]))
        wt = self.items.get(key)
        if wt is None:
            if self.frozen or torch.cuda.is_current_stream_capturing():
                return None
            wt = torch.empty(key[2], key[1], dtype=w.dtype, device=w.device)
            self.items[key] = wt
            self._rebuild()
            self.refresh()
        return wt

    def refresh(self):
        if torch.cuda.is_current_stream_capturing():
            self.frozen = True
        if self.ntiles:
            lib.ea_transpose_bf16_grouped(self.ntiles, self.tiles.data_ptr(), self.probs.data_ptr(),
                                          self.shadow.data_ptr(), stream())


def attach_transposed_shadow(shadow):
    if not WT_SHADOW or shadow is None or shadow.dtype != torch.bfloat16:
        return None
    ts = TransposedShadow(shadow)
    TSHADOWS[shadow.untyped_storage().data_ptr()] = weakref.ref(ts)
    return ts


def _transposed(w):
    if not TSHADOWS or w.dtype != torch.bfloat16 or w.dim() != 2 or w.shape[1] > WT_MAX_KIN:
        return None
    if w.stride(1) != 1 or w.stride(0) != w.shape[1] or w.shape[0] % 8 or w.shape[1] % 8:
        return None
    ref = TSHADOWS.get(w.untyped_storage().data_ptr())
    ts = None if ref is None else ref()
    if ts is None or ts.shadow.untyped_storage().data_ptr() != w.untyped_storage().data_ptr():
        return None
    return ts.get(w)


def linear_dx(dy, w, out, *, epi: Epilogue = None):
    M, N, lda = _rows(dy)
    K = w.shape[1]
    _, _, ldc = _rows(out)
    wt = _transposed(w)
    if wt is not None:
        return gemm(dy, wt, out, M=M, N=K, K=N, a_kmajor=1, b_kmajor=1, lda=lda, ldb=wt.stride(0),
                    ldc=ldc, epi=epi)
    return gemm(dy, w, out, M=M, N=K, K=N, a_kmajor=1, b_kmajor=0, lda=lda, ldb=w.stride(0),
                ldc=ldc, epi=epi)


def linear_dw(dy, x, dw, *, accumulate=False, post=None):
    R, N, lddy = _rows(dy)
    R2, K, ldx = _rows(x)
    if R != R2:
        raise HipError("row mismatch in linear_dw")
    beta = 1.0 if accumulate else 0.0
    if WGRAD_Q.active and WGRAD_Q.add(dy, x, dw, M=N, N=K, K=R, lda=lddy, ldb=ldx, ldc=dw.stride(0), beta=beta,
                                      post=post):
        return dw
    gemm(dy, x, dw, M=N, N=K, K=R, a_kmajor=0, b_kmajor=0, lda=lddy, ldb=ldx,
         ldc=dw.stride(0), epi=make_epi(beta=beta))
    if post is not None:
        post()
    return dw


def layernorm_fwd(x, gamma, beta, y, mean, rstd, eps=1e-12):
    rows, d, ldx = _rows(x)
    lib.ea_layernorm_fwd(rows, d, x.data_ptr(), ldx, gamma.data_ptr(), beta.data_ptr(), eps,
                         y.data_ptr(), dt(y), y.stride(-2) if y.dim() > 1 else d,
                         mean.data_ptr(), rstd.data_ptr(), stream())


def linear_ln(x, gamma, beta, w, out, *, epi=None, eps=1e-12):
    rows, K, ldx = _rows(x)
    N = w.shape[0]
    if epi is None:
        epi = make_epi()
    lib.ea_gemm_ln(rows, N, K, x.data_ptr(), ldx, gamma.data_ptr(), beta.data_ptr(), ctypes.c_float(eps),
                   w.data_ptr(), w.stride(0), out.data_ptr(), dt(out), out.stride(0), ctypes.byref(epi), stream())
    return out


def layernorm_bwd(dy, x, gamma, mean, rstd, dx, dgamma, dbeta, accumulate=True, drop=None):
    rows, d, ldx = _rows(x)
    _, _, lddy = _rows(dy)
    _, _, lddx = _rows(dx)
    if drop is not None:
        y, ysc, yp, yseed = drop[:4]
        ycol = drop[4] if len(drop) > 4 else None
        _, _, ldy = _rows(y)
        dargs = (y.data_ptr(), dt(y), ldy, float(ysc), float(yp), yseed & 0xFFFFFFFFFFFFFFFF,
                 0 if ycol is None else ycol.data_ptr())
    if REDUCE_Q.active and rows > 0 and dbeta.data_ptr() == dgamma.data_ptr() + 4 * d:
        vec8 = (d % 8 == 0 and d <= 1024 and lddy % 8 == 0 and ldx % 4 == 0 and lddx % 4 == 0
                and x.data_ptr() % 16 == 0 and dy.data_ptr() % 16 == 0 and dx.data_ptr() % 16 == 0
                and gamma.data_ptr() % 16 == 0)
        nparts_max = (rows + 15) // 16 if vec8 else max((rows + 15) // 16, 128)
        part = torch.empty(nparts_max * (3 if drop is not None else 2) * d, dtype=torch.float32, device=x.device)
        np_ = ctypes.c_int(0)
        if drop is not None:
            yparts = ctypes.c_int(0)
            lib.ea_layernorm_bwd_partials_drop(rows, d, dy.data_ptr(), dt(dy), lddy, x.data_ptr(), ldx,
                                               gamma.data_ptr(), mean.data_ptr(), rstd.data_ptr(), dx.data_ptr(),
                                               lddx, int(accumulate), part.data_ptr(), part.numel(),
                                               ctypes.addressof(np_), *dargs, ctypes.addressof(yparts), stream())
            if yparts.value:
                npv = np_.value
                REDUCE_Q.add_reduce(part[npv * 2 * d:], npv, d, d, ycol, accumulate=True)
        else:
            lib.ea_layernorm_bwd_partials(rows, d, dy.data_ptr(), dt(dy), lddy, x.data_ptr(), ldx, gamma.data_ptr(),
                                          mean.data_ptr(), rstd.data_ptr(), dx.data_ptr(), lddx, int(accumulate),
                                          part.data_ptr(), part.numel(), ctypes.addressof(np_), stream())
        REDUCE_Q.add_reduce(part, np_.value, 2 * d, 2 * d, dgamma, accumulate=True)
        return
    w, n = f32_ws(x.device, max(1 << 22, 1024 * d))
    if drop is not None:
        lib.ea_layernorm_bwd_drop(rows, d, dy.data_ptr(), dt(dy), lddy, x.data_ptr(), ldx, gamma.data_ptr(),
                                  mean.data_ptr(), rstd.data_ptr(), dx.data_ptr(), lddx, int(accumulate),
                                  dgamma.data_ptr(), dbeta.data_ptr(), 1, w, n, *dargs, stream())
        return
    lib.ea_layernorm_bwd(rows, d, dy.data_ptr(), dt(dy), lddy, x.data_ptr(), ldx, gamma.data_ptr(),
                         mean.data_ptr(), rstd.data_ptr(), dx.data_ptr(), lddx, int(accumulate),
                         dgamma.data_ptr(), dbeta.data_ptr(), 1, w, n, stream())


def reduce_rows(part, nparts, n, stride, out, accumulate=True):
    if REDUCE_Q.active:
        REDUCE_Q.add_reduce(part, nparts, n, stride, out, accumulate)
        return
    lib.ea_reduce_partials(nparts, n, part.data_ptr(), stride, out.data_ptr(), int(accumulate), stream())


def colsum(x, out, accumulate=True, defer=True):
    rows, n, ld = _rows(x)
    if defer and REDUCE_Q.active and REDUCE_Q.add_colsum(x, rows, n, ld, out, accumulate):
        return
    w, wn = f32_ws(x.device)
    lib.ea_colsum(rows, n, x.data_ptr(), dt(x), ld, out.data_ptr(), int(accumulate), w, wn, stream())


def batchnorm_fwd(y, gamma, beta, mean, rstd, run_mean, run_var, nbt, z, training, act,
                  eps=1e-5, momentum=0.1):
    rows, C, _ = _rows(y)
    w, wn = f32_ws(y.device, (min(rows // 16 + 1, 256) + 2) * 2 * C)
    lib.ea_batchnorm_fwd(rows, C, y.data_ptr(), gamma.data_ptr(), beta.data_ptr(), eps, momentum,
                         int(training), mean.data_ptr(), rstd.data_ptr(), ptr(run_mean), ptr(run_var),
                         ptr(nbt), act, z.data_ptr(), dt(z), w, wn, stream())


def batchnorm_bwd(dz, y, mean, rstd, gamma, beta, act, dy, dgamma, dbeta):
    rows, C, _ = _rows(y)
    w, wn = f32_ws(y.device, (min(rows // 16 + 1, 256) + 2) * 2 * C)
    lib.ea_batchnorm_bwd(rows, C, dz.data_ptr(), dt(dz), y.data_ptr(), mean.data_ptr(), rstd.data_ptr(),
                         gamma.data_ptr(), beta.data_ptr(), act, dy.data_ptr(), dgamma.data_ptr(),
                         dbeta.data_ptr(), 1, w, wn, stream())


def scale_dropout(x, y, scale=1.0, p=0.0, seed=0):
    rows, cols, ldx = _rows(x)
    _, _, ldy = _rows(y)
    lib.ea_scale_dropout(rows, cols, x.data_ptr(), dt(x), ldx, y.data_ptr(), dt(y), ldy,
                         float(scale), float(p), seed & 0xFFFFFFFFFFFFFFFF, stream())
    return y


def scale_dropout_colsum(x, y, out, scale=1.0, p=0.0, seed=0, accumulate=True):
    scale_dropout(x, y, scale=scale, p=p, seed=seed)
    with wgrad(y):
        colsum(y, out, accumulate=accumulate)
    return y


def cast(x, dtype):
    if x.dtype == dtype:
        return x
    y = torch.empty(x.shape, dtype=dtype, device=x.device)
    scale_dropout(x.reshape(-1, x.shape[-1]), y.view(-1, y.shape[-1]))
    return y


def permute3(src, dst, A, Bd, Cd, accumulate=False):
    lib.ea_permute3(A, Bd, Cd, src.data_ptr(), dt(src), dst.data_ptr(), dt(dst), int(accumulate), stream())
```

espnet-1_amd/espnet_amd/layers/conformer.py:

```python
from __future__ import annotations

import ctypes
import os

import torch
from torch import nn

from .common import (ACT_SWISH, EPI_ACT, EPI_DACT, EPI_RESID, EPI_STORE, F32, Bound, attn_bwd, attn_dmask, dbd_layout,
                     attn_fused_bwd, attn_fwd, empty, fused_attn_ok, lib, ln_bwd, ln_fwd, math, ops, rup,
                     site_seed, dv_buf, drop_arg, site_dv, REL_LATEST, REL_LEGACY)



FUSE_DW_GLU = os.environ.get("EA_FUSE_DW_GLU", "1") != "0"
GLU_IN_CONV = os.environ.get("EA_GLU_IN_CONV", "1") != "0"
BN_STATS_IN_CONV = os.environ.get("EA_BN_STATS_IN_CONV", "1") != "0"


def _glu_in_conv(K, g2, d):
    return (GLU_IN_CONV and FUSE_DW_GLU and K in (3, 5, 7, 15, 31)
            and g2.dtype == torch.bfloat16 and d % 4 == 0 and g2.data_ptr() % 8 == 0 and torch.cuda.is_available())

class PositionwiseFeedForward(nn.Module):

# ... 66 lines not shown
        self.conv_module = conv_module
        self.norm_ff = LayerNorm(size)
        self.norm_mha = LayerNorm(size)
        if feed_forward_macaron is not None:
            self.norm_ff_macaron = LayerNorm(size)
            self.ff_scale = 0.5
        else:
            self.ff_scale = 1.0
        self.norm_conv = LayerNorm(size)
        self.norm_final = LayerNorm(size)
        self.size = size
        self.dropout_rate = dropout_rate
        self.layer_idx = 0
        self._b = None

    def bind(self, arena, prefix, cd):
        self._b = Bound(arena, prefix, cd)

    @staticmethod
    def arena_groups(prefix):
        a = prefix + "self_attn."
        return [[a + "linear_q.weight", a + "linear_k.weight", a + "linear_v.weight"],
                [a + "linear_q.bias", a + "linear_k.bias", a + "linear_v.bias"]]

    def forward(self, x, pos_emb, olens, seed):
        return ConformerBlockFn.apply(x, pos_emb, olens, self, seed, self.training)


def _ffn_fwd(L, b, x_in, pre, ln_name, p, seed_in, seed_out):
    cd = b.cd
    N, d = x_in.shape
    Fh = L.feed_forward.w_1.out_features
    xn, mu, rs = ln_fwd(x_in, b, ln_name, cd)
    h = empty(N, Fh, dtype=cd, device=x_in.device)
    a = empty(N, Fh, dtype=cd, device=x_in.device)
    ops.linear(xn, b.w(pre + ".w_1.weight"), a,
               epi=ops.make_epi(EPI_ACT, bias=b.f(pre + ".w_1.bias"), act=ACT_SWISH, aux=h,
                                drop_p=p, seed=seed_in))
    x_out = empty(N, d, device=x_in.device)
    ops.linear(a, b.w(pre + ".w_2.weight"), x_out,
               epi=ops.make_epi(EPI_RESID, bias=b.f(pre + ".w_2.bias"), resid=x_in,
                                rscale=L.ff_scale, drop_p=p, seed=seed_out))
    return x_out, (xn, mu, rs, h, a)


def _ffn_bwd(L, b, dx, x_in, saved, pre, ln_name, p, seed_in, seed_out, dv_in=None, next_drop=None):
    cd = b.cd
    xn, mu, rs, h, a = saved
    N, d = dx.shape
    dv = site_dv(dx, dv_in, b.g(pre + ".w_2.bias"), L.ff_scale, p, seed_out, cd)
    with ops.wgrad(dv, a):
        ops.linear_dw(dv, a, b.g(pre + ".w_2.weight"), accumulate=True)
    dh = empty(*h.shape, dtype=cd, device=dx.device)
    ops.linear_dx(dv, b.w(pre + ".w_2.weight"), dh,
                  epi=ops.make_epi(EPI_DACT, act=ACT_SWISH, aux=h, drop_p=p, seed=seed_in))
    with ops.wgrad(dh, xn):
        ops.colsum(dh, b.g(pre + ".w_1.bias"))
        ops.linear_dw(dh, xn, b.g(pre + ".w_1.weight"), accumulate=True)
    dxn = empty(N, d, dtype=cd, device=dx.device)
    ops.linear_dx(dh, b.w(pre + ".w_1.weight"), dxn)
    ln_bwd(dxn, x_in, b, ln_name, mu, rs, dx, accumulate=True, drop=next_drop)


class ConformerBlockFn(torch.autograd.Function):
    @staticmethod
    def forward(ctx, x, pos, olens, L: EncoderLayer, seed, training):
        b = L._b
        cd = b.cd
        B, T, d = x.shape
        N = B * T
        dev = x.device
        H = L.self_attn.h
        dk = d // H
        P2 = 2 * T - 1
        p = L.dropout_rate if training else 0.0
        pa = L.self_attn.dropout_rate if training else 0.0
        li = L.layer_idx
        sd = lambda s: site_seed(seed, li, s)
        x0 = x.reshape(N, d)
        x1, s_ff1 = _ffn_fwd(L, b, x0, "feed_forward_macaron", "norm_ff_macaron", p, sd(1), sd(2))
        xn2, mu2, rs2 = ln_fwd(x1, b, "norm_mha", cd)
        A = "self_attn."
        qkv = empty(N, 3 * d, dtype=cd, device=dev)
        ops.linear(xn2, b.w(A + "linear_q.weight", A + "linear_k.weight", A + "linear_v.weight",
                            shape=(3 * d, d)), qkv,
                   epi=ops.make_epi(bias=b.f(A + "linear_q.bias", A + "linear_k.bias",
                                             A + "linear_v.bias", shape=(3 * d,))))
        mode = L.self_attn.rel_mode
        fused = fused_attn_ok(cd, dk, T, T)
        if mode == REL_LEGACY and fused:
            shift = dbd_layout(T)[0]
            pp_full = empty(shift + P2, d, dtype=cd, device=dev)
            pp_full[:shift].zero_()
            pp = pp_full[shift:]
        else:
            pp_full = None
            pp = empty(P2, d, dtype=cd, device=dev)
        if mode == REL_LEGACY:
            assert pos.shape[0] == T
            pT = empty(T, d, dtype=cd, device=dev)
            ops.linear(pos, b.w(A + "linear_pos.weight"), pT)
            lib.ea_legacy_pext(T, d, pT.data_ptr(), d, pp.data_ptr(), d, ops.dt(pp), ops.stream())
        else:
            ops.linear(pos, b.w(A + "linear_pos.weight"), pp)
        scale = 1.0 / math.sqrt(dk)
        if fused:
            O = empty(N, d, dtype=cd, device=dev)
            lse = empty(B * H * T, device=dev)
            dmask, ldm = attn_dmask(B * H * T, T, pa, dev)
            lib.ea_attn_fused_fwd2_mode(B, H, T, T, dk, qkv.data_ptr(), 3 * d, qkv[:, d:].data_ptr(), 3 * d,
# ... 58 lines not shown
                                       bn_mean.data_ptr(), bn_rstd.data_ptr(), ops.ptr(bn.running_mean),
                                       ops.ptr(bn.running_var), ops.ptr(bn.num_batches_tracked), ACT_SWISH,
                                       z.data_ptr(), ops.dt(z), ops.stream())
        else:
            ops.batchnorm_fwd(y, b.f(C + "norm.weight"), b.f(C + "norm.bias"), bn_mean, bn_rstd,
                              bn.running_mean, bn.running_var, bn.num_batches_tracked, z,
                              training, ACT_SWISH, eps=bn.eps, momentum=bn.momentum)
        x3 = empty(N, d, device=dev)
        ops.linear(z, b.w(C + "pointwise_conv2.weight", shape=(d, d)), x3,
                   epi=ops.make_epi(EPI_RESID, bias=b.f(C + "pointwise_conv2.bias"), resid=x2,
                                    drop_p=p, seed=sd(5)))
        x4, s_ff2 = _ffn_fwd(L, b, x3, "feed_forward", "norm_ff", p, sd(6), sd(7))
        out, mu5, rs5 = ln_fwd(x4, b, "norm_final", F32)
        ctx.L = L
        ctx.meta = (B, T, d, H, dk, p, pa, seed, scale, ldT, mode)
        ctx.save = (x0, x1, x2, x3, x4, s_ff1, (xn2, mu2, rs2, qkv, pp, O, s_core),
                    (xn3, mu3, rs3, g2, glu, y, z, bn_mean, bn_rstd), s_ff2, (mu5, rs5), pos, olens)
        return out.view(B, T, d)

    @staticmethod
    def backward(ctx, dout):
        L = ctx.L
        b = L._b
        cd = b.cd
        B, T, d, H, dk, p, pa, seed, scale, ldT, mode = ctx.meta
        (x0, x1, x2, x3, x4, s_ff1, s_att, s_conv, s_ff2, (mu5, rs5), pos, olens) = ctx.save
        ctx.save = None
        li = L.layer_idx
        sd = lambda s: site_seed(seed, li, s)
        N = B * T
        dev = dout.device
        P2 = 2 * T - 1
        dx = empty(N, d, device=dev)
        dv_ff2 = dv_buf(N, d, cd, dev)
        ln_bwd(dout.reshape(N, d).contiguous(), x4, b, "norm_final", mu5, rs5, dx, accumulate=False,
               drop=drop_arg(dv_ff2, L.ff_scale, p, sd(7), b.g("feed_forward.w_2.bias")))
        dv_conv = dv_buf(N, d, cd, dev)
        _ffn_bwd(L, b, dx, x3, s_ff2, "feed_forward", "norm_ff", p, sd(6), sd(7), dv_in=dv_ff2,
                 next_drop=drop_arg(dv_conv, 1.0, p, sd(5), b.g("conv_module.pointwise_conv2.bias")))
        C = "conv_module."
        K = L.conv_module.kernel_size
        xn3, mu3, rs3, g2, glu, y, z, bn_mean, bn_rstd = s_conv
        dv = site_dv(dx, dv_conv, b.g(C + "pointwise_conv2.bias"), 1.0, p, sd(5), cd)
        with ops.wgrad(dv, z):
            ops.linear_dw(dv, z, b.g(C + "pointwise_conv2.weight", shape=(d, d)), accumulate=True)
        dz = empty(N, d, dtype=cd, device=dev)
        ops.linear_dx(dv, b.w(C + "pointwise_conv2.weight", shape=(d, d)), dz)
        dy = empty(N, d, device=dev)
        ops.batchnorm_bwd(dz, y, bn_mean, bn_rstd, b.f(C + "norm.weight"), b.f(C + "norm.bias"),
                          ACT_SWISH, dy, b.g(C + "norm.weight"), b.g(C + "norm.bias"))
        dg2 = empty(N, 2 * d, dtype=cd, device=dev)
        fuse = FUSE_DW_GLU and K in (3, 5, 7, 15, 31) and g2.dtype == torch.bfloat16
        if fuse:
            w, wn = ops.f32_ws(dev, B * ((T + 31) // 32) * d * (K + 1) + 1024)
            lib.ea_dwconv_glu_bwd(B, T, d, K, ops.ptr(glu), b.f(C + "depthwise_conv.weight").data_ptr(),
                                  dy.data_ptr(), g2.data_ptr(), dg2.data_ptr(),
                                  b.g(C + "depthwise_conv.weight").data_ptr(),
                                  b.g(C + "depthwise_conv.bias").data_ptr(), 1, w, wn, ops.stream())
        else:
            if glu is None:
                glu = empty(N, d, device=dev)
                lib.ea_glu_fwd(N, d, g2.data_ptr(), ops.dt(g2), glu.data_ptr(), 0, ops.stream())
            dglu = empty(N, d, device=dev)
            w, wn = ops.f32_ws(dev, B * ((T + 31) // 32) * d * (K + 1) + 1024)
            lib.ea_dwconv_bwd(B, T, d, K, glu.data_ptr(), b.f(C + "depthwise_conv.weight").data_ptr(),
                              dy.data_ptr(), dglu.data_ptr(), b.g(C + "depthwise_conv.weight").data_ptr(),
                              b.g(C + "depthwise_conv.bias").data_ptr(), 1, w, wn, ops.stream())
            lib.ea_glu_bwd(N, d, g2.data_ptr(), ops.dt(g2), dglu.data_ptr(), dg2.data_ptr(), ops.stream())
        with ops.wgrad(dg2, xn3):
            ops.colsum(dg2, b.g(C + "pointwise_conv1.bias"))
            ops.linear_dw(dg2, xn3, b.g(C + "pointwise_conv1.weight", shape=(2 * d, d)), accumulate=True)
        dxn3 = empty(N, d, dtype=cd, device=dev)
        ops.linear_dx(dg2, b.w(C + "pointwise_conv1.weight", shape=(2 * d, d)), dxn3)
        dv_att = dv_buf(N, d, cd, dev)
        ln_bwd(dxn3, x2, b, "norm_conv", mu3, rs3, dx, accumulate=True,
               drop=drop_arg(dv_att, 1.0, p, sd(4), b.g("self_attn.linear_out.bias")))
        A = "self_attn."
        xn2, mu2, rs2, qkv, pp, O, s_core = s_att
        dv = site_dv(dx, dv_att, b.g(A + "linear_out.bias"), 1.0, p, sd(4), cd)
        with ops.wgrad(dv, O):
            ops.linear_dw(dv, O, b.g(A + "linear_out.weight"), accumulate=True)
        dO = empty(N, d, dtype=cd, device=dev)
        ops.linear_dx(dv, b.w(A + "linear_out.weight"), dO)
        dqkv = empty(N, 3 * d, dtype=cd, device=dev)
        ldbd, shift = rup(P2, 8), 0
        if s_core[0] == "fused":
            _, lse, dmask, ldm, pp_full = s_core
            legacy = mode == REL_LEGACY
            shift, ldbd = dbd_layout(T)
            dbd = empty(H * B * T * ldbd, dtype=cd, device=dev)
            qv = empty(N, d, dtype=cd, device=dev)
            nqb = (T + 63) // 64
            part = empty(2 * B * nqb * d, device=dev)
            attn_fused_bwd(B=B, H=H, T1=T, T2=T, q=qkv, ldq=3 * d, k=qkv[:, d:], ldk=3 * d, v=qkv[:, 2 * d:],
                           ldv=3 * d, bu=b.f(A + "pos_bias_u"), bv=b.f(A + "pos_bias_v"), pp=pp, ldp=d,
                           klen=olens, causal=False, scale=scale, p=pa, seed=sd(3), O=O, ldo=d, lse=lse, dO=dO,
                           lddo=d, dq=dqkv, lddq=3 * d, dk=dqkv[:, d:], lddk=3 * d, dv=dqkv[:, 2 * d:],
                           lddv=3 * d, dbd=dbd, ldbd=ldbd, part=part, ldpart=d, qv_out=qv, ldqv=d, dmask=dmask,
                           ldm=ldm, flags=2 if legacy else 1 | 2, rel_mode=mode)
            ops.reduce_rows(part[:B * nqb * d], B * nqb, d, d, b.g(A + "pos_bias_u", shape=(d,)))
            if legacy:
                raw = dbd
                dbd = empty(H * B * T * ldbd, dtype=cd, device=dev)
                lib.ea_attn_legacy_band(H * B, T, raw.data_ptr(), dbd.data_ptr(), ldbd, ops.stream())
                del raw
                dqv = empty(N, d, dtype=cd, device=dev)
                ops.gemm(dbd, pp_full, dqv, M=T, N=dk, K=shift + P2, a_kmajor=1, b_kmajor=0, lda=ldbd, ldb=d, ldc=d,
                         batch=B, nh=H, sA=(T * ldbd, B * T * ldbd), sB=(0, dk), sC=(T * d, dk), splitk=False)
                ops.colsum(dqv, b.g(A + "pos_bias_v", shape=(d,)))
                lib.ea_add_2d(N, d, dqv.data_ptr(), ops.dt(dqv), d, dqkv.data_ptr(), ops.dt(dqkv), 3 * d, 1.0,
                              ops.stream())
            else:
                ops.reduce_rows(part[B * nqb * d:], B * nqb, d, d, b.g(A + "pos_bias_v", shape=(d,)))
        else:
            _, qu, qv, P, Pd = s_core
            dbd = empty(H * B * T * ldbd, dtype=cd, device=dev)
            attn_bwd(dO, qu, qkv[:, d:], qkv[:, 2 * d:], P, Pd, ldT, B=B, H=H, T1=T, T2=T, dk=dk,
                     ldq=d, ldk=3 * d, ldv=3 * d, scale=scale, p=pa, seed=sd(3), cd=cd,
                     dq=dqkv, lddq=3 * d, dk_=dqkv[:, d:], lddk=3 * d, dv=dqkv[:, 2 * d:], lddv=3 * d,
                     dbd=dbd, ldbd=ldbd, rel_mode=mode)
# ... 41 lines not shown
```

espnet-1_amd/espnet_amd/layers/decoder.py:

```python
from __future__ import annotations

import math

import torch
from torch import nn

from .common import (ACT_RELU, EPI_ACT, EPI_DACT, EPI_RESID, EPI_STORE, F32, Bound, attn_bwd,
                     attn_dmask, attn_fused_bwd, attn_fwd, empty, fused_attn_ok, lib, ln_bwd, ln_fwd, ops,
                     site_seed, dv_buf, drop_arg, site_dv)


def _mha_fwd(q, k, v, *, B, H, T1, T2, dk, ldq, ldk, ldv, klen, causal, scale, p, seed, cd):
    if fused_attn_ok(cd, dk, T1, T2):
        O = empty(B * T1, H * dk, dtype=cd, device=q.device)
        lse = empty(B * H * T1, device=q.device)
        dmask, ldm = attn_dmask(B * H * T1, T2, p, q.device)
        lib.ea_attn_fused_fwd2(B, H, T1, T2, dk, q.data_ptr(), ldq, k.data_ptr(), ldk, v.data_ptr(), ldv,
                               None, None, None, 0, klen.data_ptr(), int(causal), scale, float(p), seed,
                               O.data_ptr(), H * dk, lse.data_ptr(), ops.ptr(dmask), ldm, ops.stream())
        return O, ("fused", O, lse, dmask, ldm)
    O, P, Pd, ldT = attn_fwd(q, k, v, B=B, H=H, T1=T1, T2=T2, dk=dk, ldq=ldq, ldk=ldk, ldv=ldv, klen=klen,
                             causal=causal, scale=scale, p=p, seed=seed, cd=cd)
    return O, ("unfused", P, Pd, ldT)

# ... 147 lines not shown
                       epi=ops.make_epi(EPI_ACT, bias=b.f(ff + "w_1.bias"), act=ACT_RELU, aux=h,
                                        drop_p=p, seed=sd(l, 5)))
            x3 = empty(N, d, device=dev)
            ops.linear(a, b.w(ff + "w_2.weight"), x3,
                       epi=ops.make_epi(EPI_RESID, bias=b.f(ff + "w_2.bias"), resid=x2,
                                        drop_p=p, seed=sd(l, 6)))
            saved.append((x, x1, x2, (xn1, mu1, rs1, qkv, O1, st1),
                          (xn2, mu2, rs2, q2, O2, st2), (xn3, mu3, rs3, h, a)))
            x = x3
        xf, muf, rsf = ln_fwd(x, b, "after_norm", cd)
        logits = empty(N, V, device=dev)
        ops.linear(xf, b.w("output_layer.weight"), logits,
                   epi=ops.make_epi(bias=b.f("output_layer.bias")))
        ctx.dec = dec
        ctx.meta = (B, Tm, L, d, H, dk, nb, p, p_sa, p_src, p_pos, seed, scale)
        ctx.save = (mem, kv, ys_in, saved, x, xf, muf, rsf, hlens, ys_in_lens)
        return logits.view(B, L, V)

    @staticmethod
    def backward(ctx, dlogits):
        dec = ctx.dec
        b = dec._b
        cd = b.cd
        B, Tm, L, d, H, dk, nb, p, p_sa, p_src, p_pos, seed, scale = ctx.meta
        mem, kv, ys_in, saved, xlast, xf, muf, rsf, hlens, ys_in_lens = ctx.save
        ctx.save = None
        sd = lambda l, s: site_seed(seed, 100 + l, s)
        N, Nm = B * L, B * Tm
        V = dlogits.shape[-1]
        dev = dlogits.device
        dlog = ops.cast(dlogits.reshape(N, V).contiguous(), cd)
        with ops.wgrad(dlog, xf):
            ops.colsum(dlog, b.g("output_layer.bias"))
            ops.linear_dw(dlog, xf, b.g("output_layer.weight"), accumulate=True)
        dxf = empty(N, d, dtype=cd, device=dev)
        ops.linear_dx(dlog, b.w("output_layer.weight"), dxf)
        dx = empty(N, d, device=dev)
        dv_ff = dv_buf(N, d, cd, dev) if nb > 0 else None
        ln_bwd(dxf, xlast, b, "after_norm", muf, rsf, dx, accumulate=False,
               drop=None if dv_ff is None else
               drop_arg(dv_ff, 1.0, p, sd(nb - 1, 6), b.g(f"decoders.{nb - 1}.feed_forward.w_2.bias")))
        ldkv = 2 * d * nb
        dkv = empty(Nm, ldkv, dtype=cd, device=dev)
        for l in reversed(range(nb)):
            n = f"decoders.{l}."
            sa, xa, ff = n + "self_attn.", n + "src_attn.", n + "feed_forward."
            x0, x1, x2, s1, s2, s3 = saved[l]
            xn3, mu3, rs3, h, a = s3
            dv = site_dv(dx, dv_ff, b.g(ff + "w_2.bias"), 1.0, p, sd(l, 6), cd)
            with ops.wgrad(dv, a):
                ops.linear_dw(dv, a, b.g(ff + "w_2.weight"), accumulate=True)
            fork = ops.fork_event() if l < nb - 1 else None
            dh = empty(*h.shape, dtype=cd, device=dev)
            ops.linear_dx(dv, b.w(ff + "w_2.weight"), dh,
                          epi=ops.make_epi(EPI_DACT, act=ACT_RELU, aux=h, drop_p=p, seed=sd(l, 5)))
            if fork is not None:
                ops.flush_wgrad_side(after=fork)
            with ops.wgrad(dh, xn3):
                ops.colsum(dh, b.g(ff + "w_1.bias"))
                ops.linear_dw(dh, xn3, b.g(ff + "w_1.weight"), accumulate=True)
            dxn = empty(N, d, dtype=cd, device=dev)
            ops.linear_dx(dh, b.w(ff + "w_1.weight"), dxn)
            dv_src = dv_buf(N, d, cd, dev)
            ln_bwd(dxn, x2, b, n + "norm3", mu3, rs3, dx, accumulate=True,
                   drop=drop_arg(dv_src, 1.0, p, sd(l, 4), b.g(xa + "linear_out.bias")))
            xn2, mu2, rs2, q2, O2, st2 = s2
            dv = site_dv(dx, dv_src, b.g(xa + "linear_out.bias"), 1.0, p, sd(l, 4), cd)
            with ops.wgrad(dv, O2):
                ops.linear_dw(dv, O2, b.g(xa + "linear_out.weight"), accumulate=True)
            dO = empty(N, d, dtype=cd, device=dev)
            ops.linear_dx(dv, b.w(xa + "linear_out.weight"), dO)
            dq = empty(N, d, dtype=cd, device=dev)
            _mha_bwd(st2, dO, q2, kv[:, 2 * d * l:], kv[:, 2 * d * l + d:], B=B, H=H, T1=L, T2=Tm, dk=dk,
                     ldq=d, ldk=ldkv, ldv=ldkv, klen=hlens, causal=False, scale=scale, p=p_src,
                     seed=sd(l, 3), cd=cd, dq=dq, lddq=d, dk_=dkv[:, 2 * d * l:], lddk=ldkv,
                     dv=dkv[:, 2 * d * l + d:], lddv=ldkv)
            with ops.wgrad(dq, xn2):
                ops.colsum(dq, b.g(xa + "linear_q.bias"))
                ops.linear_dw(dq, xn2, b.g(xa + "linear_q.weight"), accumulate=True)
            dxn = empty(N, d, dtype=cd, device=dev)
            ops.linear_dx(dq, b.w(xa + "linear_q.weight"), dxn)
            dv_self = dv_buf(N, d, cd, dev)
            ln_bwd(dxn, x1, b, n + "norm2", mu2, rs2, dx, accumulate=True,
                   drop=drop_arg(dv_self, 1.0, p, sd(l, 2), b.g(sa + "linear_out.bias")))
            xn1, mu1, rs1, qkv, O1, st1 = s1
            dv = site_dv(dx, dv_self, b.g(sa + "linear_out.bias"), 1.0, p, sd(l, 2), cd)
            with ops.wgrad(dv, O1):
                ops.linear_dw(dv, O1, b.g(sa + "linear_out.weight"), accumulate=True)
            dO = empty(N, d, dtype=cd, device=dev)
            ops.linear_dx(dv, b.w(sa + "linear_out.weight"), dO)
            dqkv = empty(N, 3 * d, dtype=cd, device=dev)
            _mha_bwd(st1, dO, qkv, qkv[:, d:], qkv[:, 2 * d:], B=B, H=H, T1=L, T2=L, dk=dk,
                     ldq=3 * d, ldk=3 * d, ldv=3 * d, klen=ys_in_lens, causal=True, scale=scale, p=p_sa,
                     seed=sd(l, 1), cd=cd, dq=dqkv, lddq=3 * d, dk_=dqkv[:, d:], lddk=3 * d,
                     dv=dqkv[:, 2 * d:], lddv=3 * d)
            wn = (sa + "linear_q.weight", sa + "linear_k.weight", sa + "linear_v.weight")
            bn = (sa + "linear_q.bias", sa + "linear_k.bias", sa + "linear_v.bias")
            with ops.wgrad(dqkv, xn1):
                ops.colsum(dqkv, b.g(*bn, shape=(3 * d,)))
                ops.linear_dw(dqkv, xn1, b.g(*wn, shape=(3 * d, d)), accumulate=True)
            dxn = empty(N, d, dtype=cd, device=dev)
            ops.linear_dx(dqkv, b.w(*wn, shape=(3 * d, d)), dxn)
            dv_ff = dv_buf(N, d, cd, dev) if l > 0 else None
            ln_bwd(dxn, x0, b, n + "norm1", mu1, rs1, dx, accumulate=True,
                   drop=None if dv_ff is None else
                   drop_arg(dv_ff, 1.0, p, sd(l - 1, 6), b.g(f"decoders.{l - 1}.feed_forward.w_2.bias")))
        pe = dec.embed[1]
        lib.ea_embed_bwd(N, d, ys_in.data_ptr(), dx.data_ptr(), pe.xscale, p_pos, sd(0, 0),
                         b.g("embed.0.weight").data_ptr(), ops.stream())
        kvw, kvb = _kv_names(nb)
        with ops.wgrad(dkv, mem):
            ops.colsum(dkv, b.g(*kvb, shape=(ldkv,)))
# ... 6 lines not shown
```

espnet-1_amd/espnet_amd/layers/subsampling.py:

```python
from __future__ import annotations

import ctypes
import math
import os

import torch
from torch import nn

from .._lib import CONV_DGRAD, CONV_FWD, CONV_WGRAD, GEMM_PIPE, ConvGeo
from .common import (ACT_RELU, EPI_ACT, EPI_DACT, EPI_STORE, F32, Bound, empty, lib, ops, rup)


def phase_geo(B, T1, F1, T2, F2, C, mode, a=0, e=0, zero=0):
    g = ConvGeo()
    g.mode, g.B, g.T2, g.F2, g.C, g.P = mode, B, T2, F2, C, B * T2 * F2
    nI = ((T1 + 1) // 2, T1 // 2)
    nJ = ((F1 + 1) // 2, F1 // 2)
    g.nI[0], g.nI[1] = nI
    g.nJ[0], g.nJ[1] = nJ
    rows = [B * nI[0] * nJ[0], B * nI[0] * nJ[1], B * nI[1] * nJ[0], B * nI[1] * nJ[1]]
    off = 0
    for i in range(4):
        g.plane[i] = off * C
        off += rows[i]
# ... 160 lines not shown
        x1p = empty(P1 + 64, C, dtype=cd, device=dev)
        x1p[P1:].zero_()
        pos1 = (torch.empty(P1 * C // 8, dtype=torch.uint8, device=dev)
                if training and FUSE_CONV1_WGRAD and CONV1_POS_BITS else None)
        lib.ea_conv1_fwd2(B, T, Fin, C, feats.data_ptr(), b.f("conv.0.weight").data_ptr(),
                          b.f("conv.0.bias").data_ptr(), x1p.data_ptr(), ops.dt(x1p),
                          0 if pos1 is None else pos1.data_ptr(), ops.stream())
        w2 = empty(C, 9 * C, dtype=cd, device=dev)
        ops.permute3(b.f("conv.2.weight"), w2, C * C // 64, 64, 9)
        x2 = empty(P2, C, dtype=cd, device=dev)
        geo, _, _, _ = phase_geo(B, T1, F1, T2, F2, C, CONV_FWD)
        probe = ops.PROBE
        if probe is not None:
            probe.begin("conv2_gemm")
        epi = ops.make_epi(EPI_ACT, bias=b.f("conv.2.bias"), act=ACT_RELU)
        ws = ops.splitk_ws(dev)
        lib.ea_gemm_conv(ctypes.byref(geo), 1, 1, P2, C, 9 * C, x1p.data_ptr(), C, w2.data_ptr(), 9 * C,
                         x2.data_ptr(), ops.dt(x2), C, ctypes.byref(epi), ws.data_ptr(), ws.numel(), ops.stream())
        if probe is not None:
            probe.end("conv2_gemm")
        wl = empty(C, F2 * C, dtype=cd, device=dev)
        ops.permute3(b.f("out.0.weight"), wl, C, C, F2)
        p = pe.dropout_rate if training else 0.0
        y = _out_linear(x2.view(B * T2, F2 * C), wl, b, pe, p, seed, B, T2, C)
        ctx.m = m
        ctx.implicit = True
        ctx.meta = (B, T, Fin, T1, F1, T2, F2, p, seed)
        ctx.save = (feats, x1p, w2, x2, wl, pos1)
        return y.view(B, T2, C)

    @staticmethod
    def _backward_implicit(ctx, dy):
        m = ctx.m
        b = m._b
        cd = b.cd
        B, T, Fin, T1, F1, T2, F2, p, seed = ctx.meta
        feats, x1p, w2, x2, wl, pos1 = ctx.save
        ctx.save = None
        C = m.odim
        dev = dy.device
        P1, P2 = B * T1 * F1, B * T2 * F2
        dv = empty(B * T2, C, dtype=cd, device=dev)
        ops.scale_dropout_colsum(dy.reshape(B * T2, C).contiguous(), dv, b.g("out.0.bias"), scale=m.out[1].xscale,
                                 p=p, seed=seed)
        x2r = x2.view(B * T2, F2 * C)
        with ops.wgrad(dv, x2):
            dwl = empty(C, F2 * C, device=dev)
            gw = b.g("out.0.weight")
            ops.linear_dw(dv, x2r, dwl, accumulate=False,
                          post=lambda: ops.permute3(dwl, gw, C, F2, C, accumulate=True))
        K2 = rup(P2, 64)
        dx2 = empty(P2 + 128, C, dtype=cd, device=dev)
        dx2[P2:].zero_()
        ops.linear_dx(dv, wl, dx2[:P2].view(B * T2, F2 * C), epi=ops.make_epi(EPI_DACT, act=ACT_RELU, aux=x2r))
        ws_side = None
        with ops.wgrad(dx2, x1p, launches=True):
            ops.colsum(dx2[:P2], b.g("conv.2.bias"))
            dw2 = empty(C, 9 * C, device=dev)
            geo, _, _, _ = phase_geo(B, T1, F1, T2, F2, C, CONV_WGRAD, zero=P1 * C)
            epi = ops.make_epi()
            ws_side = ops.splitk_ws(dev)
            lib.ea_gemm_conv(ctypes.byref(geo), 0, 0, C, 9 * C, K2, dx2.data_ptr(), C, x1p.data_ptr(), C,
                             dw2.data_ptr(), ops.dt(dw2), 9 * C, ctypes.byref(epi), ws_side.data_ptr(),
                             ws_side.numel(), ops.stream())
            ops.permute3(dw2, b.g("conv.2.weight"), C, 9, C, accumulate=True)
        ws = ops.splitk_ws(dev)
        fuse = FUSE_CONV1_WGRAD
        kmaj = DGRAD_KMAJOR and fuse and pos1 is not None and MERGED_DGRAD
        if kmaj:
            w2t = empty(C, 9 * C, dtype=cd, device=dev)
            ops.permute3(b.f("conv.2.weight"), w2t, 1, C, 9 * C)
        else:
            w2t = empty(9, C, C, dtype=cd, device=dev)
            ops.permute3(b.f("conv.2.weight"), w2t, 1, C * C, 9)
        if fuse:
            _, _, _, rows_all = phase_geo(B, T1, F1, T2, F2, C, CONV_DGRAD)
            part = empty(sum((r + 255) // 256 for r in rows_all) * 10 * C, device=dev)
            tile0 = 0
        else:
            dx1p = empty(P1, C, dtype=cd, device=dev)
        if fuse and pos1 is not None and MERGED_DGRAD:
            geo, _, _, _ = phase_geo(B, T1, F1, T2, F2, C, CONV_DGRAD, zero=P2 * C)
            epi = ops.make_epi(EPI_DACT, act=ACT_RELU)
            lib.ea_gemm_conv_w1b_all(ctypes.byref(geo), C, dx2.data_ptr(), C, w2t.data_ptr(), 9 * C if kmaj else C,
                                     ctypes.byref(epi),
                                     feats.data_ptr(), T, Fin, part.data_ptr(), pos1.data_ptr(), ops.stream())
            tile0 = sum((r + 255) // 256 for r in rows_all if r)
        else:
            for a in (0, 1):
                for e in (0, 1):
                    geo, nI, nJ, rows = phase_geo(B, T1, F1, T2, F2, C, CONV_DGRAD, a=a, e=e, zero=P2 * C)
                    Mc = rows[a * 2 + e]
                    if Mc == 0:
                        continue
                    ntaps = (1 if a else 2) * (1 if e else 2)
                    o = geo.plane[a * 2 + e] // C
                    aux = x1p[o:o + Mc]
                    epi = ops.make_epi(EPI_DACT, act=ACT_RELU, aux=aux)
                    if fuse and pos1 is None:
                        lib.ea_gemm_conv_w1(ctypes.byref(geo), Mc, C, ntaps * C, dx2.data_ptr(), C, w2t.data_ptr(), C,
                                            ctypes.byref(epi), feats.data_ptr(), T, Fin,
                                            part.data_ptr() + 4 * tile0 * 10 * C, ops.stream())
                        tile0 += (Mc + 255) // 256
                    elif fuse:
                        lib.ea_gemm_conv_w1b(ctypes.byref(geo), Mc, C, ntaps * C, dx2.data_ptr(), C, w2t.data_ptr(), C,
                                             ctypes.byref(epi), feats.data_ptr(), T, Fin,
                                             part.data_ptr() + 4 * tile0 * 10 * C, pos1.data_ptr() + o * (C // 8),
                                             ops.stream())
                        tile0 += (Mc + 255) // 256
                    else:
                        lib.ea_gemm_conv(ctypes.byref(geo), 1, 0, Mc, C, ntaps * C, dx2.data_ptr(), C, w2t.data_ptr(),
                                         C, dx1p[o:o + Mc].data_ptr(), ops.dt(dx1p), C, ctypes.byref(epi),
                                         ws.data_ptr(), ws.numel(), ops.stream())
        if fuse:
            lib.ea_conv1_wgrad_reduce(tile0, C, part.data_ptr(), b.g("conv.0.weight").data_ptr(),
                                      b.g("conv.0.bias").data_ptr(), ops.stream())
        else:
            with ops.wgrad(dx1p, feats, launches=True):
                w, wn = ops.f32_ws(dev, 1024 * 10 * C)
                lib.ea_conv1_wgrad(B, T, Fin, C, feats.data_ptr(), dx1p.data_ptr(), ops.dt(dx1p),
                                   b.g("conv.0.weight").data_ptr(), b.g("conv.0.bias").data_ptr(), w, wn, ops.stream())
        ops.grad_ready(b)
        return None, None, None, None, None

    @staticmethod
    def backward(ctx, dy):
        if ctx.implicit:
            return SubsampleFn._backward_implicit(ctx, dy)
        m = ctx.m
        b = m._b
        cd = b.cd
        B, T, Fin, T1, F1, T2, F2, p, seed = ctx.meta
        col1, x1, col2, w2, x2, wl = ctx.save
        ctx.save = None
        C = m.odim
        dev = dy.device
        dv = empty(B * T2, C, dtype=cd, device=dev)
        ops.scale_dropout_colsum(dy.reshape(B * T2, C).contiguous(), dv, b.g("out.0.bias"), scale=m.out[1].xscale,
                                 p=p, seed=seed)
        x2r = x2.view(B * T2, F2 * C)
        with ops.wgrad(dv, x2):
            dwl = empty(C, F2 * C, device=dev)
            gw = b.g("out.0.weight")
            ops.linear_dw(dv, x2r, dwl, accumulate=False,
                          post=lambda: ops.permute3(dwl, gw, C, F2, C, accumulate=True))
        dx2 = empty(B * T2, F2 * C, dtype=cd, device=dev)
        ops.linear_dx(dv, wl, dx2, epi=ops.make_epi(EPI_DACT, act=ACT_RELU, aux=x2r))
        dx2 = dx2.view(-1, C)
        with ops.wgrad(dx2, col2):
            ops.colsum(dx2, b.g("conv.2.bias"))
            dw2 = empty(C, 9 * C, device=dev)
            g2 = b.g("conv.2.weight")
            ops.linear_dw(dx2, col2, dw2, accumulate=False,
                          post=lambda: ops.permute3(dw2, g2, C, 9, C, accumulate=True))
        dcol2 = empty(*col2.shape, dtype=cd, device=dev)
        ops.linear_dx(dx2, w2, dcol2)
        del col2
        dx1 = empty(*x1.shape, dtype=cd, device=dev)
        lib.ea_col2im_conv2(B, T1, F1, C, dcol2.data_ptr(), ops.dt(dcol2), x1.data_ptr(), dx1.data_ptr(),
                            ops.dt(dx1), ops.stream())
        del dcol2
        with ops.wgrad(dx1, col1, launches=True):
            ops.colsum(dx1, b.g("conv.0.bias"))
            ops.gemm(dx1, col1, b.g("conv.0.weight", shape=(C, 9)), M=C, N=9, K=dx1.shape[0],
                     a_kmajor=0, b_kmajor=0, lda=C, ldb=16, ldc=9, epi=ops.make_epi(beta=1.0))
        ops.grad_ready(b)
        return None, None, None, None, None
```

espnet-1_amd/espnet_amd/layers/transformer.py:

```python
from __future__ import annotations

import math

import torch
from torch import nn

from .common import (ACT_RELU, EPI_ACT, EPI_DACT, EPI_RESID, Bound, empty, ln_bwd, ln_fwd, ops, site_dv,
                     site_seed)
from .conformer import LayerNorm
from .decoder import _mha_bwd, _mha_fwd


class TransformerEncoderLayer(nn.Module):

    def __init__(self, size, self_attn, feed_forward, dropout_rate, normalize_before=True, concat_after=False,
                 stochastic_depth_rate=0.0):
        super().__init__()
        if not normalize_before or concat_after or stochastic_depth_rate > 0:
            raise NotImplementedError("only normalize_before=True, concat_after=False, "
                                      "stochastic_depth_rate=0 are implemented")
        self.self_attn = self_attn
        self.feed_forward = feed_forward
        self.norm1 = LayerNorm(size)
        self.norm2 = LayerNorm(size)
# ... 26 lines not shown
        cd = b.cd
        B, T, d = x.shape
        N = B * T
        dev = x.device
        H = L.self_attn.h
        dk = d // H
        p = L.dropout_rate if training else 0.0
        pa = L.self_attn.dropout_rate if training else 0.0
        p_ff = L.feed_forward.dropout_rate if training else 0.0
        sd = lambda s: site_seed(seed, 50 + L.layer_idx, s)
        scale = 1.0 / math.sqrt(dk)
        x0 = x.reshape(N, d)
        xn1, mu1, rs1 = ln_fwd(x0, b, "norm1", cd)
        qkv = empty(N, 3 * d, dtype=cd, device=dev)
        ops.linear(xn1, b.w(*_QKV_W, shape=(3 * d, d)), qkv, epi=ops.make_epi(bias=b.f(*_QKV_B, shape=(3 * d,))))
        O, st = _mha_fwd(qkv, qkv[:, d:], qkv[:, 2 * d:], B=B, H=H, T1=T, T2=T, dk=dk, ldq=3 * d, ldk=3 * d,
                         ldv=3 * d, klen=olens, causal=getattr(L, "causal", False), scale=scale, p=pa, seed=sd(1), cd=cd)
        x1 = empty(N, d, device=dev)
        ops.linear(O, b.w("self_attn.linear_out.weight"), x1,
                   epi=ops.make_epi(EPI_RESID, bias=b.f("self_attn.linear_out.bias"), resid=x0, drop_p=p,
                                    seed=sd(2)))
        xn2, mu2, rs2 = ln_fwd(x1, b, "norm2", cd)
        Fh = L.feed_forward.w_1.out_features
        h = empty(N, Fh, dtype=cd, device=dev)
        a = empty(N, Fh, dtype=cd, device=dev)
        ops.linear(xn2, b.w("feed_forward.w_1.weight"), a,
                   epi=ops.make_epi(EPI_ACT, bias=b.f("feed_forward.w_1.bias"), act=ACT_RELU, aux=h, drop_p=p_ff,
                                    seed=sd(3)))
        x2 = empty(N, d, device=dev)
        ops.linear(a, b.w("feed_forward.w_2.weight"), x2,
                   epi=ops.make_epi(EPI_RESID, bias=b.f("feed_forward.w_2.bias"), resid=x1, drop_p=p, seed=sd(4)))
        ctx.L = L
        ctx.meta = (B, T, d, H, dk, p, pa, p_ff, seed, scale)
        ctx.save = (x0, x1, (xn1, mu1, rs1, qkv, O, st), (xn2, mu2, rs2, h, a), olens)
        return x2.view(B, T, d)

    @staticmethod
    def backward(ctx, dout):
        L = ctx.L
        b = L._b
        cd = b.cd
        B, T, d, H, dk, p, pa, p_ff, seed, scale = ctx.meta
        x0, x1, s_att, s_ff, olens = ctx.save
        ctx.save = None
        sd = lambda s: site_seed(seed, 50 + L.layer_idx, s)
        N = B * T
        dev = dout.device
        dx = dout.reshape(N, d).contiguous().clone()
        xn2, mu2, rs2, h, a = s_ff
        dv = site_dv(dx, None, b.g("feed_forward.w_2.bias"), 1.0, p, sd(4), cd)
        with ops.wgrad(dv, a):
            ops.linear_dw(dv, a, b.g("feed_forward.w_2.weight"), accumulate=True)
        dh = empty(*h.shape, dtype=cd, device=dev)
        ops.linear_dx(dv, b.w("feed_forward.w_2.weight"), dh,
                      epi=ops.make_epi(EPI_DACT, act=ACT_RELU, aux=h, drop_p=p_ff, seed=sd(3)))
        with ops.wgrad(dh, xn2):
            ops.colsum(dh, b.g("feed_forward.w_1.bias"))
            ops.linear_dw(dh, xn2, b.g("feed_forward.w_1.weight"), accumulate=True)
        dxn = empty(N, d, dtype=cd, device=dev)
        ops.linear_dx(dh, b.w("feed_forward.w_1.weight"), dxn)
        ln_bwd(dxn, x1, b, "norm2", mu2, rs2, dx, accumulate=True)
        xn1, mu1, rs1, qkv, O, st = s_att
        dv = site_dv(dx, None, b.g("self_attn.linear_out.bias"), 1.0, p, sd(2), cd)
        with ops.wgrad(dv, O):
            ops.linear_dw(dv, O, b.g("self_attn.linear_out.weight"), accumulate=True)
        dO = empty(N, d, dtype=cd, device=dev)
        ops.linear_dx(dv, b.w("self_attn.linear_out.weight"), dO)
        dqkv = empty(N, 3 * d, dtype=cd, device=dev)
        _mha_bwd(st, dO, qkv, qkv[:, d:], qkv[:, 2 * d:], B=B, H=H, T1=T, T2=T, dk=dk, ldq=3 * d, ldk=3 * d,
                 ldv=3 * d, klen=olens, causal=getattr(L, "causal", False), scale=scale, p=pa, seed=sd(1), cd=cd, dq=dqkv, lddq=3 * d,
                 dk_=dqkv[:, d:], lddk=3 * d, dv=dqkv[:, 2 * d:], lddv=3 * d)
        with ops.wgrad(dqkv, xn1):
            ops.colsum(dqkv, b.g(*_QKV_B, shape=(3 * d,)))
            ops.linear_dw(dqkv, xn1, b.g(*_QKV_W, shape=(3 * d, d)), accumulate=True)
        dxn = empty(N, d, dtype=cd, device=dev)
        ops.linear_dx(dqkv, b.w(*_QKV_W, shape=(3 * d, d)), dxn)
        ln_bwd(dxn, x0, b, "norm1", mu1, rs1, dx, accumulate=True)
        ops.grad_ready(b)
        return dx.view(B, T, d), None, None, None, None
```

include/espnet_amd.h:

```cpp
#ifndef ESPNET_AMD_H
#define ESPNET_AMD_H

#include <stddef.h>

#ifdef __cplusplus
extern "C" {
#endif

enum { EA_F32 = 0, EA_BF16 = 1 };
enum { EA_OK = 0, EA_ERR_BAD_ARG = 1000 };
enum { EA_ACT_NONE = 0, EA_ACT_SWISH = 1, EA_ACT_RELU = 2 };

enum { EA_EPI_STORE = 0, EA_EPI_ACT = 1, EA_EPI_RESID = 2, EA_EPI_DACT = 3 };

typedef struct ea_epilogue {
  int kind;
  int act;
  float alpha, beta, post_scale, rscale, drop_p;
  unsigned long long seed;
  const float* bias;
  void* aux;
  int aux_dtype;
  long ldaux;
  const float* resid;
  long ldr;
} ea_epilogue;

int ea_gemm(int dtype, int a_kmajor, int b_kmajor, int M, int N, int K,
            const void* A, long lda, long sAb, long sAh,
            const void* B, long ldb, long sBb, long sBh,
            int batch, int nh,
            void* C, int c_dtype, long ldc, long sCb, long sCh,
            const ea_epilogue* epi, float* workspace, long ws_elems, void* stream);


enum { EA_CONV_FWD = 1, EA_CONV_DGRAD = 2, EA_CONV_WGRAD = 3 };
typedef struct ea_conv_geo {
  int mode;
  int B, T2, F2, C, P;
  int nI[2], nJ[2];
  int a, e;
  long plane[4];
  long zero;
} ea_conv_geo;
int ea_gemm_conv(const ea_conv_geo* geo, int a_kmajor, int b_kmajor, int M, int N, int K,
                 const void* A, long lda, const void* B, long ldb, void* C, int c_dtype, long ldc,
                 const ea_epilogue* epi, float* workspace, long ws_elems, void* stream);
int ea_gemm_conv_w1(const ea_conv_geo* geo, int M, int N, int K, const void* A, long lda, const void* B,
                    long ldb, const ea_epilogue* epi, const float* x, int T, int Fin, float* part,
                    void* stream);
int ea_gemm_conv_w1b(const ea_conv_geo* geo, int M, int N, int K, const void* A, long lda, const void* B,
                     long ldb, const ea_epilogue* epi, const float* x, int T, int Fin, float* part,
                     const unsigned char* pos, void* stream);
int ea_gemm_conv_w1b_all(const ea_conv_geo* geo, int N, const void* A, long lda, const void* B, long ldb,
                         const ea_epilogue* epi, const float* x, int T, int Fin, float* part,
                         const unsigned char* pos, void* stream);
int ea_conv1_wgrad_reduce(int ntiles, int C, const float* part, float* dw, float* dbias, void* stream);

int ea_gemm_set_pipeline(int stages);

int ea_gemm_set_tile(int bm, int bn);
int ea_gemm_set_pipe(int on);
int ea_gemm_set_k128(int mode, int slots);
int ea_gemm_set_skinny(int max_m);
int ea_gemm_ln(int M, int N, int K, const float* x, long ldx, const float* gamma, const float* beta, float eps,
               const void* W, long ldw, void* C, int c_dtype, long ldc, const ea_epilogue* epi, void* stream);

typedef struct ea_group_gemm {
  const void* A;
  const void* B;
  float* C;
  long lda, ldb, ldc;
  int M, N, K;
  float beta;
} ea_group_gemm;
int ea_gemm_grouped(int a_kmajor, int b_kmajor, int n, const ea_group_gemm* probs, void* ws, long ws_bytes,
                    void* stream);
int ea_gemm_grouped_ws_bytes(int n, long ntiles, long* bytes);
int ea_gemm_grouped_set_xcd_chunk(int chunk);

int ea_gemm_set_probe(unsigned long long* slots);
int ea_gemm_set_diag(unsigned long long* buf);
int ea_phase_stamp(unsigned long long* state, float* ring, int cap, int phase, const float* extra, void* stream);
struct ea_opt_state;
int ea_phase_stamp_opt(unsigned long long* state, float* ring, int cap, int phase, const struct ea_opt_state* opt,
                       void* stream);
int ea_probe_begin(unsigned long long* slots, void* stream);
int ea_probe_end(unsigned long long* slots, void* stream);
int ea_debug_spin(long ns, void* stream);
void* ea_guard_malloc(size_t size, int device, void* stream);
void ea_guard_free(void* ptr, size_t size, int device, void* stream);


int ea_layernorm_fwd(int rows, int d, const float* x, long ldx, const float* gamma,
                     const float* beta, float eps, void* y, int y_dtype, long ldy,
                     float* mean, float* rstd, void* stream);

int ea_layernorm_bwd(int rows, int d, const void* dy, int dy_dtype, long lddy, const float* x,
                     long ldx, const float* gamma, const float* mean, const float* rstd,
                     float* dx, long lddx, int accumulate, float* dgamma, float* dbeta,
                     int accumulate_params, float* workspace, long ws_elems, void* stream);

int ea_reduce_partials(int nparts, int n, const float* part, long stride, float* out,
                       int accumulate, void* stream);

int ea_colsum(int rows, int n, const void* x, int x_dtype, long ld, float* out, int accumulate,
              float* workspace, long ws_elems, void* stream);

int ea_layernorm_bwd_partials(int rows, int d, const void* dy, int dy_dtype, long lddy, const float* x,
                              long ldx, const float* gamma, const float* mean, const float* rstd,
                              float* dx, long lddx, int accumulate, float* part, long part_elems,
                              int* nparts, void* stream);

int ea_layernorm_bwd_drop(int rows, int d, const void* dy, int dy_dtype, long lddy, const float* x,
                          long ldx, const float* gamma, const float* mean, const float* rstd, float* dx,
                          long lddx, int accumulate, float* dgamma, float* dbeta, int accumulate_params,
                          float* workspace, long ws_elems, void* y, int y_dtype, long ldy, float yscale,
                          float p, unsigned long long seed, float* ycol, void* stream);
int ea_layernorm_bwd_partials_drop(int rows, int d, const void* dy, int dy_dtype, long lddy,
                                   const float* x, long ldx, const float* gamma, const float* mean,
                                   const float* rstd, float* dx, long lddx, int accumulate, float* part,
                                   long part_elems, int* nparts, void* y, int y_dtype, long ldy,
                                   float yscale, float p, unsigned long long seed, float* ycol,
                                   int* ycol_parts, void* stream);

typedef struct ea_colsum_prob {
  const void* x;
  float* part;
  long ld;
  int rows, n, dtype, rpp;
} ea_colsum_prob;
typedef struct ea_reduce_prob {
  const float* part;
  float* out;
  long stride;
  int nparts, n, accumulate;
} ea_reduce_prob;
int ea_colsum_grouped(int n, const ea_colsum_prob* probs, void* ws, long ws_bytes, void* stream);
int ea_reduce_grouped(int n, const ea_reduce_prob* probs, void* ws, long ws_bytes, void* stream);
int ea_grouped_table_bytes(int n, long* colsum_bytes, long* reduce_bytes);

int ea_batchnorm_fwd(int rows, int C, const float* y, const float* gamma, const float* beta,
                     float eps, float momentum, int training, float* mean, float* rstd,
                     float* running_mean, float* running_var, long long* num_batches_tracked,
                     int act, void* z, int z_dtype, float* workspace, long ws_elems, void* stream);

int ea_batchnorm_fwd_parts(int rows, int C, const float* y, const float* part, int nparts, const float* shift,
                           const float* gamma, const float* beta, float eps, float momentum, float* mean,
                           float* rstd, float* running_mean, float* running_var, long long* num_batches_tracked,
                           int act, void* z, int z_dtype, void* stream);

int ea_batchnorm_bwd(int rows, int C, const void* dz, int dz_dtype, const float* y, const float* mean,
                     const float* rstd, const float* gamma, const float* beta, int act, float* dy,
                     float* dgamma, float* dbeta, int accumulate_params, float* workspace,
                     long ws_elems, void* stream);


int ea_utterance_mvn(int B, int T, int F, const float* x, const long long* lens, float* y, void* stream);
int ea_utterance_mvn_ws_bytes(int B, int T, int F, long* bytes);
int ea_utterance_mvn2(int B, int T, int F, const float* x, const long long* lens, float* y, void* ws,
                      long ws_bytes, void* stream);

int ea_stft_frames(int B, long Ns, int nF, int n_fft, int hop, int center, const float* x,
                   const float* window, float* frames, void* stream);
int ea_power_spectrum(long M, int nF, int nbins, const float* spec, long ld_spec, const long long* flens,
                      float* power, long ld_power, void* stream);
int ea_logmel_mvn(long M, int nF, int n_mels, const float* mel, long ld_mel, const long long* flens,
                  const float* mean, const float* std, float* y, void* stream);
int ea_global_mvn(int B, int T, int D, const float* x, const long long* lens, const float* mean,
                  const float* std, float* y, void* stream);

int ea_specaug(int B, int T, int F, const float* x, const long long* lengths, const int* warp, int per_utt,
               const int* fmask, int nf, const int* tmask, int nt, float* y, void* stream);

int ea_subsample_lens(int B, int T, const long long* ilens, long long* olens, void* stream);

int ea_add_sos_eos(int B, int L, const long long* ys, long ldys, const long long* ylens, int sos,
                   int eos, int ignore_id, long long* ys_in, long long* ys_out,
                   long long* ys_in_lens, void* stream);

int ea_scale_dropout(long rows, int cols, const void* x, int x_dtype, long ldx, void* y,
                     int y_dtype, long ldy, float scale, float p, unsigned long long seed,
                     void* stream);

int ea_scale_dropout_colsum(long rows, int cols, const float* x, long ldx, void* y, int y_dtype, long ldy,
                            float scale, float p, unsigned long long seed, float* colsum, int accumulate,
                            float* workspace, long ws_elems, void* stream);

int ea_add_2d(long rows, int cols, const void* x, int x_dtype, long ldx, void* y, int y_dtype,
              long ldy, float alpha, void* stream);

int ea_permute3(int A, int Bd, int Cd, const void* src, int src_dtype, void* dst, int dst_dtype,
                int accumulate, void* stream);

int ea_im2col_conv1(int B, int T, int F, const float* x, void* col, int col_dtype, void* stream);
int ea_im2col_conv2(int B, int T1, int F1, int C, const void* x1, void* col, int dtype, void* stream);
int ea_col2im_conv2(int B, int T1, int F1, int C, const void* dcol, int dcol_dtype, const void* x1,
                    void* dx1, int dtype, void* stream);

int ea_conv1_fwd(int B, int T, int F, int C, const float* x, const float* w, const float* bias,
                 void* x1p, int dtype, void* stream);
int ea_conv1_fwd2(int B, int T, int F, int C, const float* x, const float* w, const float* bias,
                  void* x1p, int dtype, unsigned char* pos, void* stream);
int ea_conv1_wgrad(int B, int T, int F, int C, const float* x, const void* dh, int dtype, float* dw,
                   float* dbias, float* workspace, long ws_elems, void* stream);

int ea_glu_fwd(long rows, int C, const void* x, int x_dtype, void* y, int y_dtype, void* stream);
int ea_glu_bwd(long rows, int C, const void* x, int x_dtype, const float* dy, void* dx, void* stream);

int ea_dwconv_fwd(int B, int T, int C, int K, const float* x, const float* w, const float* bias,
                  float* y, void* stream);
int ea_dwconv_bwd(int B, int T, int C, int K, const float* x, const float* w, const float* dy,
                  float* dx, float* dw, float* dbias, int accumulate_params, float* workspace,
                  long ws_elems, void* stream);
int ea_dwconv_glu_bwd(int B, int T, int C, int K, const float* x, const float* w, const float* dy,
                      const void* g2, void* dg2, float* dw, float* dbias, int accumulate_params,
                      float* workspace, long ws_elems, void* stream);
int ea_dwconv_fwd_glu(int B, int T, int C, int K, const void* g2, const float* w, const float* bias,
                      float* y, void* stream);
int ea_dwconv_fwd_glu_stats(int B, int T, int C, int K, const void* g2, const float* w, const float* bias,
                            float* y, float* part, void* stream);
int ea_dwconv_stats_parts(int B, int T, int* nparts);
int ea_add_pos_bias(long N, int H, int dk, const void* q, long ldq, const float* u, const float* v,
                    void* qu, void* qv, int dtype, void* stream);

int ea_embed_fwd(long rows, int d, int L, const long long* tok, const float* E, float xscale,
                 const float* pe, float p, unsigned long long seed, float* y, void* stream);
int ea_add_pe_dropout(long rows, int d, int L, const float* pe, float p, unsigned long long seed, float* y,
                      void* stream);
int ea_embed_bwd(long rows, int d, const long long* tok, const float* dy, float xscale, float p,
                 unsigned long long seed, float* dE, void* stream);

int ea_set_rng_salt(const unsigned long long* salt);
int ea_rng_advance(unsigned long long* salt, void* stream);

int ea_argmax_rows(long rows, int V, const float* x, long ld, long long* out, void* stream);


int ea_attn_softmax_fwd(int B, int H, int T1, int T2, float scale, const float* S, long ldS,
                        const float* BD, long ldBD, const long long* klen, int causal, float p,
                        unsigned long long seed, float* P, long ldP, void* Pd, int pd_dtype,
                        long ldPd, void* stream);

int ea_attn_softmax_bwd(int B, int H, int T1, int T2, float scale, const float* dPd, long ldd,
                        const float* P, long ldP, float p, unsigned long long seed, void* dS,
                        int ds_dtype, long ldS, void* dBD, long ldBD, void* stream);

enum { EA_REL_LATEST = 0, EA_REL_LEGACY = 1 };
int ea_attn_softmax_fwd_mode(int B, int H, int T1, int T2, float scale, const float* S, long ldS,
                             const float* BD, long ldBD, const long long* klen, int causal, float p,
                             unsigned long long seed, float* P, long ldP, void* Pd, int pd_dtype,
                             long ldPd, int rel_mode, void* stream);
int ea_attn_softmax_bwd_mode(int B, int H, int T1, int T2, float scale, const float* dPd, long ldd,
                             const float* P, long ldP, float p, unsigned long long seed, void* dS,
                             int ds_dtype, long ldS, void* dBD, long ldBD, int rel_mode, void* stream);
int ea_legacy_pext(int T, int d, const void* p, long ldp, void* pext, long ldx, int dtype, void* stream);
int ea_legacy_pext_fold(int T, int d, const void* dpext, long ldx, void* dp, long ldp, int dtype,
                        void* stream);

int ea_attn_fused_fwd(int B, int H, int T1, int T2, int dk, const void* q, long ldq, const void* k,
                      long ldk, const void* v, long ldv, const float* bu, const float* bv,
                      const void* pp, long ldp, const long long* klen, int causal, float scale, float p,
                      unsigned long long seed, void* o, long ldo, float* lse, void* stream);
int ea_attn_fused_fwd2(int B, int H, int T1, int T2, int dk, const void* q, long ldq, const void* k,
                       long ldk, const void* v, long ldv, const float* bu, const float* bv,
                       const void* pp, long ldp, const long long* klen, int causal, float scale, float p,
                       unsigned long long seed, void* o, long ldo, float* lse, unsigned* dmask, int ldm,
                       void* stream);
int ea_attn_fused_fwd2_mode(int B, int H, int T1, int T2, int dk, const void* q, long ldq, const void* k,
                            long ldk, const void* v, long ldv, const float* bu, const float* bv,
// ... 157 lines not shown
```

Baseline: 1912 utterances/s.

## Fuse bias-gradient column sums into DACT GEMM epilogue and defer dwconv partial reductions

The activation-backward GEMM epilogue now also writes per-64-row column partial sums of its bf16 output, so the separate colsum pass over dh for the FFN w_1 bias and the subsampling conv bias is dropped. Depthwise-conv backward gets partials-only entry points, so their weight and bias reductions can be queued into the grouped reducer. That reducer is widened to 64 columns with float4 loads and gains a transposed-output mode. The risk is extra registers and shuffles in the GEMM epilogue; it also falls back silently when the alignment or tile preconditions fail.

```diff
diff --git a/espnet-1_amd/csrc/elementwise.hip b/espnet-1_amd/csrc/elementwise.hip
--- a/espnet-1_amd/csrc/elementwise.hip
+++ b/espnet-1_amd/csrc/elementwise.hip
@@ -1156,6 +1156,30 @@
   return 0;
 }
 
+static int dwconv_bwd_k_launch(int B, int T, int C, int K, const float* x, const float* w, const float* dy, float* dx,
+                               float* part, long part_elems, int* nparts, void* stream) {
+  const int nblkr = B * ea_cdiv(T, 4 * DW_R);
+  dim3 gridr(nblkr, ea_cdiv(C, DW_CT));
+  EA_CHECK_ARG(part && (long)nblkr * C * (K + 1) <= part_elems);
+  hipStream_t st = (hipStream_t)stream;
+  switch (K) {
+#define EA_DWB(KK) case KK: hipLaunchKernelGGL((dwconv_bwd_k_kernel<KK, DW_R>), gridr, dim3(256), 0, st, B, T, C, x, w, dy, dx, part); break;
+    EA_DWB(3) EA_DWB(5) EA_DWB(7) EA_DWB(15) EA_DWB(31)
+#undef EA_DWB
+    default: return EA_ERR_BAD_ARG;
+  }
+  EA_LAUNCH_CHECK();
+  *nparts = nblkr;
+  return 0;
+}
+
+extern "C" int ea_dwconv_bwd_partials(int B, int T, int C, int K, const float* x, const float* w, const float* dy,
+                                      float* dx, float* part, long part_elems, int* nparts, void* stream) {
+  EA_ENTRY();
+  EA_CHECK_ARG(nparts != nullptr);
+  return dwconv_bwd_k_launch(B, T, C, K, x, w, dy, dx, part, part_elems, nparts, stream);
+}
+
 extern "C" int ea_dwconv_bwd(int B, int T, int C, int K, const float* x, const float* w, const float* dy, float* dx,
                              float* dw, float* dbias, int accumulate_params, float* workspace, long ws_elems,
                              void* stream) {
@@ -1164,17 +1188,10 @@
   const int nblk = B * ea_cdiv(T, DW_TT);
   dim3 grid(nblk, ea_cdiv(C, DW_CT));
   if (K == 3 || K == 5 || K == 7 || K == 15 || K == 31) {
-    const int nblkr = B * ea_cdiv(T, 4 * DW_R);
-    dim3 gridr(nblkr, ea_cdiv(C, DW_CT));
+    int nblkr = 0;
     const long rowlen = (long)C * (K + 1);
-    EA_CHECK_ARG((long)nblkr * rowlen <= ws_elems);
-    hipStream_t st = (hipStream_t)stream;
-    switch (K) {
-#define EA_DWB(KK) case KK: hipLaunchKernelGGL((dwconv_bwd_k_kernel<KK, DW_R>), gridr, dim3(256), 0, st, B, T, C, x, w, dy, dx, workspace); break;
-      EA_DWB(3) EA_DWB(5) EA_DWB(7) EA_DWB(15) EA_DWB(31)
-#undef EA_DWB
-    }
-    EA_LAUNCH_CHECK();
+    int rc0 = dwconv_bwd_k_launch(B, T, C, K, x, w, dy, dx, workspace, ws_elems, &nblkr, stream);
+    if (rc0) return rc0;
     int rc = ea_reduce_partials_tr(nblkr, C * K, workspace, rowlen, dw, accumulate_params, C, K, stream);
     if (rc || !dbias) return rc;
     return ea_reduce_partials(nblkr, C, workspace + (long)C * K, rowlen, dbias, accumulate_params, stream);
@@ -1237,18 +1254,16 @@
   return 0;
 }
 
-extern "C" int ea_dwconv_glu_bwd(int B, int T, int C, int K, const float* x, const float* w, const float* dy,
-                                 const void* g2, void* dg2, float* dw, float* dbias, int accumulate_params,
-                                 float* workspace, long ws_elems, void* stream) {
-  EA_ENTRY();
-  EA_CHECK_ARG((K == 3 || K == 5 || K == 7 || K == 15 || K == 31) && g2 && dg2 && dw && dbias);
+static int dwconv_glu_bwd_launch(int B, int T, int C, int K, const float* x, const float* w, const float* dy,
+                                 const void* g2, void* dg2, float* workspace, long ws_elems, int* nparts,
+                                 void* stream) {
+  EA_CHECK_ARG((K == 3 || K == 5 || K == 7 || K == 15 || K == 31) && g2 && dg2 && workspace);
   EA_CHECK_ARG(x != nullptr || (C % 4 == 0 && ((uintptr_t)g2 % 8) == 0));
   const int nblkr = B * ea_cdiv(T, 4 * DW_R);
   dim3 gridr(nblkr, ea_cdiv(C, DW_CT));
   const long rowlen = (long)C * (K + 1);
   EA_CHECK_ARG((long)nblkr * rowlen <= ws_elems);
   hipStream_t st = (hipStream_t)stream;
-  const bool adj = dbias == dw + (long)C * K;
   switch (K) {
 #define EA_DWB(KK)                                                                                              \
   case KK:                                                                                                      \
@@ -1263,6 +1278,28 @@
 #undef EA_DWB
   }
   EA_LAUNCH_CHECK();
+  *nparts = nblkr;
+  return 0;
+}
+
+extern "C" int ea_dwconv_glu_bwd_partials(int B, int T, int C, int K, const float* x, const float* w, const float* dy,
+                                          const void* g2, void* dg2, float* part, long part_elems, int* nparts,
+                                          void* stream) {
+  EA_ENTRY();
+  EA_CHECK_ARG(nparts != nullptr);
+  return dwconv_glu_bwd_launch(B, T, C, K, x, w, dy, g2, dg2, part, part_elems, nparts, stream);
+}
+
+extern "C" int ea_dwconv_glu_bwd(int B, int T, int C, int K, const float* x, const float* w, const float* dy,
+                                 const void* g2, void* dg2, float* dw, float* dbias, int accumulate_params,
+                                 float* workspace, long ws_elems, void* stream) {
+  EA_ENTRY();
+  EA_CHECK_ARG(dw && dbias);
+  int nblkr = 0;
+  int rc0 = dwconv_glu_bwd_launch(B, T, C, K, x, w, dy, g2, dg2, workspace, ws_elems, &nblkr, stream);
+  if (rc0) return rc0;
+  const long rowlen = (long)C * (K + 1);
+  const bool adj = dbias == dw + (long)C * K;
   if (adj) return ea_reduce_partials_tr(nblkr, (int)rowlen, workspace, rowlen, dw, accumulate_params, C, K, stream);
   int rc = ea_reduce_partials_tr(nblkr, C * K, workspace, rowlen, dw, accumulate_params, C, K, stream);
   if (rc) return rc;
diff --git a/espnet-1_amd/csrc/gemm.hip b/espnet-1_amd/csrc/gemm.hip
--- a/espnet-1_amd/csrc/gemm.hip
+++ b/espnet-1_amd/csrc/gemm.hip
@@ -67,6 +67,7 @@
 }
 
 int g_force_bm = 0, g_force_bn = 0;
+thread_local int g_colsum_rows = 0;
 void choose_tile(GemmP& p, int a_k, long nz) {
   struct Cfg { int bm, bn, occ; double t0, rcu; bool ak_only; };
   static const Cfg cfgs[] = {{256, 256, 1, 12.4, 4.49, false}, {128, 128, 2, 8.3, 2.9, false},
@@ -208,6 +209,12 @@
   EA_ENTRY();
   EA_CHECK_ARG(max_m >= 0 && max_m <= 64);
   g_gemm_skinny = max_m;
+  return 0;
+}
+
+extern "C" int ea_gemm_colsum_rows(int* rows) {
+  EA_CHECK_ARG(rows != nullptr);
+  *rows = g_colsum_rows;
   return 0;
 }
 
@@ -242,6 +249,7 @@
   p.nh = nh;
   p.C = C; p.c_dtype = c_dtype; p.ldc = ldc; p.sCb = sCb; p.sCh = sCh;
   p.epi = *epi;
+  g_colsum_rows = 0;
   p.ws = workspace;
   p.salt = ea_g_rng_salt;
   p.stamp = g_probe;
@@ -324,6 +332,14 @@
   }
   p.splitk = splitk;
   p.kchunk = kchunk;
+  if (p.epi.colsum_part) {
+    const bool ok = epi->kind == EA_EPI_DACT && dtype == EA_BF16 && p.lds && p.vec8 && splitk == 1 && nz == 1 &&
+                    p.g.mode == 0 && !w1part && p.bm >= 128 && p.epi.ldpart % 4 == 0 && p.epi.ldpart >= N &&
+                    ((uintptr_t)p.epi.colsum_part % 16) == 0 &&
+                    (p.bm == 256 || k128 || !(g_gemm_pipe & 2));
+    if (ok)g_colsum_rows = ea_cdiv(M, 64);
+    else p.epi.colsum_part = nullptr;
+  }
   static const bool trace = std::getenv("EA_GEMM_TRACE") != nullptr;
   if (trace)
     std::fprintf(stderr, "[ea_gemm] M=%d N=%d K=%d ak=%d bk=%d nz=%d tile=%dx%d%s splitk=%d epi=%d geo=%d lds=%d\n", M,
@@ -370,6 +386,7 @@
   p.nh = 1; p.splitk = 1; p.kchunk = K;
   p.C = C; p.c_dtype = c_dtype; p.ldc = ldc;
   p.epi = *epi;
+  p.epi.colsum_part = nullptr;
   p.salt = ea_g_rng_salt;
   const int ce = c_dtype == EA_BF16 ? 2 : 4;
   bool vc = (N % 4 == 0) && ldc % 4 == 0 && ((uintptr_t)C % (4 * ce)) == 0;
@@ -428,6 +445,7 @@
   p.nh = 1; p.splitk = 1;
   p.C = nullptr; p.c_dtype = EA_BF16; p.ldc = N;
   p.epi = *epi;
+  p.epi.colsum_part = nullptr;
   p.salt = ea_g_rng_salt;
   p.stamp = g_probe;
   p.diag = g_diag;
diff --git a/espnet-1_amd/csrc/gemm_kern.h b/espnet-1_amd/csrc/gemm_kern.h
--- a/espnet-1_amd/csrc/gemm_kern.h
+++ b/espnet-1_amd/csrc/gemm_kern.h
@@ -332,9 +332,10 @@
     v[2 * q + 1] *= (h >> 16) >= k.thr ? k.sc : 0.f;
   }
 }
-template <int KIND>
+template <int KIND, bool CSUM = false>
 EA_DEV void epi_eight_pre(const GemmP& p, const EpiK& k, int z, int zb, int zh, int row, int col,
-                          const float (&acc)[8], const float (&bias)[8], bool has_o, const float (&o)[8]) {
+                          const float (&acc)[8], const float (&bias)[8], bool has_o, const float (&o)[8],
+                          float* cs = nullptr) {
   const ea_epilogue& e = p.epi;
   const long cidx = zb * p.sCb + zh * p.sCh + (long)row * p.ldc + col;
   const uint64_t didx = ((uint64_t)z * p.M + row) * (uint64_t)p.N + col;
@@ -363,7 +364,22 @@
   } else {
     drop8k(k, didx, v);
     act_bwd_mul_n<8>(e.act, v, o);
-    st8(p.C, cidx, p.c_dtype, v);
+    if constexpr (CSUM) {
+      if (p.c_dtype == EA_BF16) {
+        union { uint4 u; bf16 b[8]; } t;
+#pragma unroll
+        for (int c = 0; c < 8; ++c) t.b[c] = (bf16)v[c];
+        *(uint4*)((bf16*)p.C + cidx) = t.u;
+#pragma unroll
+        for (int c = 0; c < 8; ++c) cs[c] += (float)t.b[c];
+      } else {
+        st8(p.C, cidx, EA_F32, v);
+#pragma unroll
+        for (int c = 0; c < 8; ++c) cs[c] += v[c];
+      }
+    } else {
+      st8(p.C, cidx, p.c_dtype, v);
+    }
   }
 }
 
@@ -596,7 +612,26 @@
   return ti;
 }
 
-template <int KIND, int MI, int NJ>
+template <int KIND, int HB8, bool CSUM>
+EA_DEV void epi_rows8(const GemmP& p, const EpiK& k, int z, int zb, int zh, const float* t, int row0, int lr0, int lc8,
+                      int col, float* slab, const float (&bias)[8], bool reads, const float (&o)[HB8][8],
+                      float (&cs)[8]) {
+#pragma unroll
+  for (int it = 0; it < HB8; ++it) {
+    const int lr = lr0 + it * 8, row = row0 + it * 8;
+    const float4 f0 = *(const float4*)(t + lr * EPI_LDT + lc8), f1 = *(const float4*)(t + lr * EPI_LDT + lc8 + 4);
+    if (row >= p.M || col >= p.N) continue;
+    if (slab) {
+      *(float4*)(slab + (long)row * p.N + col) = f0;
+      *(float4*)(slab + (long)row * p.N + col + 4) = f1;
+      continue;
+    }
+    const float v[8] = {f0.x, f0.y, f0.z, f0.w, f1.x, f1.y, f1.z, f1.w};
+    epi_eight_pre<KIND, CSUM>(p, k, z, zb, zh, row, col, v, bias, reads, o[it], cs);
+  }
+}
+
+template <int KIND, int MI, int NJ, bool CS = true>
 EA_DEV void epi_wave(const GemmP& p, const EpiK& k, char* smem, int z, int zb, int zh, int r0, int c0, int lane,
                      int w, const f32x4 (&acc)[MI][NJ], int sk = 0) {
   constexpr int RC = MI < 4 ? MI : 4;
@@ -675,10 +710,13 @@
     constexpr int NG8 = RC * 2;
     constexpr int HB8 = NG8 < 4 ? NG8 : 4;
     const int lc8 = (lane & 7) * 8, rl = lane >> 3;
+    bool cs_on = false;
+    if constexpr (CS && KIND == EA_EPI_DACT && RC == 4) cs_on = p.epi.colsum_part != nullptr && !slab;
 #pragma unroll
     for (int ch = 0; ch < NCH; ++ch) {
       transpose(ch);
       const int rb = ch_rb(ch), col = c0 + (ch % (NJ / 4)) * 64 + lc8;
+      float cs[8] = {0.f, 0.f, 0.f, 0.f, 0.f, 0.f, 0.f, 0.f};
       float bias[8] = {0.f, 0.f, 0.f, 0.f, 0.f, 0.f, 0.f, 0.f};
       if (!slab && KIND != EA_EPI_DACT && p.epi.bias && col < p.N) {
         const float4 b0 = *(const float4*)(p.epi.bias + col), b1 = *(const float4*)(p.epi.bias + col + 4);
@@ -700,18 +738,20 @@
               ld8(src, sbase + (long)min(rb + (h0 + it) * 8 + rl, p.M - 1) * sld + cl, EA_F32, o[it]);
           }
         }
-#pragma unroll
-        for (int it = 0; it < HB8; ++it) {
-          const int lr = (h0 + it) * 8 + rl, row = rb + lr;
-          const float4 f0 = *(const float4*)(t + lr * EPI_LDT + lc8), f1 = *(const float4*)(t + lr * EPI_LDT + lc8 + 4);
-          if (row >= p.M || col >= p.N) continue;
-          if (slab) {
-            *(float4*)(slab + (long)row * p.N + col) = f0;
-            *(float4*)(slab + (long)row * p.N + col + 4) = f1;
-            continue;
-          }
-          const float v[8] = {f0.x, f0.y, f0.z, f0.w, f1.x, f1.y, f1.z, f1.w};
-          epi_eight_pre<KIND>(p, k, z, zb, zh, row, col, v, bias, reads, o[it]);
+        if (cs_on) epi_rows8<KIND, HB8, true>(p, k, z, zb, zh, t, rb + h0 * 8 + rl, h0 * 8 + rl, lc8, col, slab, bias, reads, o, cs);
+        else epi_rows8<KIND, HB8, false>(p, k, z, zb, zh, t, rb + h0 * 8 + rl, h0 * 8 + rl, lc8, col, slab, bias, reads, o, cs);
+      }
+      if (cs_on && rb < p.M) {
+#pragma unroll
+        for (int c = 0; c < 8; ++c) {
+          cs[c] += __shfl_xor(cs[c], 8);
+          cs[c] += __shfl_xor(cs[c], 16);
+          cs[c] += __shfl_xor(cs[c], 32);
+        }
+        if (rl == 0 && col < p.N) {
+          float* d = p.epi.colsum_part + (long)(rb >> 6) * p.epi.ldpart + col;
+          *(float4*)d = make_float4(cs[0], cs[1], cs[2], cs[3]);
+          *(float4*)(d + 4) = make_float4(cs[4], cs[5], cs[6], cs[7]);
         }
       }
     }
@@ -994,7 +1034,7 @@
     case EA_EPI_STORE: epi_wave<EA_EPI_STORE, MI, NJ>(p, ek, smem, z, zb, zh, m0 + wm, n0 + wn, lane, w, acc, sk); break;
     case EA_EPI_ACT: epi_wave<EA_EPI_ACT, MI, NJ>(p, ek, smem, z, zb, zh, m0 + wm, n0 + wn, lane, w, acc, sk); break;
     case EA_EPI_RESID: epi_wave<EA_EPI_RESID, MI, NJ>(p, ek, smem, z, zb, zh, m0 + wm, n0 + wn, lane, w, acc, sk); break;
-    default: epi_wave<EA_EPI_DACT, MI, NJ>(p, ek, smem, z, zb, zh, m0 + wm, n0 + wn, lane, w, acc, sk); break;
+    default: epi_wave<EA_EPI_DACT, MI, NJ, MODE == 0>(p, ek, smem, z, zb, zh, m0 + wm, n0 + wn, lane, w, acc, sk); break;
   }
   probe_end(p);
 }
@@ -1630,7 +1670,7 @@
     case EA_EPI_STORE: epi_wave<EA_EPI_STORE, MI, 4>(p, ek, smem, z, zb, zh, m0 + wm, n0 + wn, lane, w, acc, sk); break;
     case EA_EPI_ACT: epi_wave<EA_EPI_ACT, MI, 4>(p, ek, smem, z, zb, zh, m0 + wm, n0 + wn, lane, w, acc, sk); break;
     case EA_EPI_RESID: epi_wave<EA_EPI_RESID, MI, 4>(p, ek, smem, z, zb, zh, m0 + wm, n0 + wn, lane, w, acc, sk); break;
-    default: epi_wave<EA_EPI_DACT, MI, 4>(p, ek, smem, z, zb, zh, m0 + wm, n0 + wn, lane, w, acc, sk); break;
+    default: epi_wave<EA_EPI_DACT, MI, 4, MODE == 0>(p, ek, smem, z, zb, zh, m0 + wm, n0 + wn, lane, w, acc, sk); break;
   }
   if (p.diag) {
     __syncthreads();
diff --git a/espnet-1_amd/csrc/reduce.hip b/espnet-1_amd/csrc/reduce.hip
--- a/espnet-1_amd/csrc/reduce.hip
+++ b/espnet-1_amd/csrc/reduce.hip
@@ -14,6 +14,7 @@
   float* out;
   long stride;
   int nparts, n, accumulate, item0;
+  int tr_rows, tr_cols;
 };
 
 constexpr int CHUNK = 40;
@@ -97,32 +98,69 @@
   if (cc < q.n) q.part[(long)rb * q.n + cc] = (red[0][t] + red[1][t]) + (red[2][t] + red[3][t]);
 }
 
-constexpr int RP_CW = 16, RP_PL = 16;
+constexpr int RP_CW = 64, RP_PL = 16;
 __global__ __launch_bounds__(256) void reduce_grouped_kernel(const ReduceProbD* __restrict__ table, int nprob) {
   __shared__ double red[RP_PL][RP_CW];
   const int pi = find_prob(table, nprob, blockIdx.x);
   const ReduceProbD q = table[pi];
-  const int cx = threadIdx.x % RP_CW, py = threadIdx.x / RP_CW;
-  const int c = (blockIdx.x - q.item0) * RP_CW + cx;
-  double a = 0.0;
-  if (c < q.n) {
-    int p = py;
-    for (; p + 7 * RP_PL < q.nparts; p += 8 * RP_PL) {
-      float v[8];
-#pragma unroll
-      for (int j = 0; j < 8; ++j) v[j] = q.part[(long)(p + RP_PL * j) * q.stride + c];
-#pragma unroll
-      for (int j = 0; j < 8; ++j) a += v[j];
-    }
-    for (; p < q.nparts; p += RP_PL) a += q.part[(long)p * q.stride + c];
-  }
-  red[py][cx] = a;
+  const int cx = threadIdx.x % 16, py = threadIdx.x / 16;
+  const int c0 = (blockIdx.x - q.item0) * RP_CW;
+  const bool vec = (((uintptr_t)q.part & 15) | (q.stride & 3) | (q.n & 3)) == 0;
+  double a[4] = {0.0, 0.0, 0.0, 0.0};
+  if (vec) {
+    const int c = c0 + cx * 4;
+    if (c < q.n) {
+      const float* x = q.part + c;
+      int p = py;
+      for (; p + 7 * RP_PL < q.nparts; p += 8 * RP_PL) {
+        float4 v[8];
+#pragma unroll
+        for (int j = 0; j < 8; ++j) v[j] = *(const float4*)(x + (long)(p + RP_PL * j) * q.stride);
+#pragma unroll
+        for (int j = 0; j < 8; ++j) {
+          a[0] += v[j].x; a[1] += v[j].y; a[2] += v[j].z; a[3] += v[j].w;
+        }
+      }
+      if (p < q.nparts) {
+        float4 v[7];
+#pragma unroll
+        for (int j = 0; j < 7; ++j) v[j] = *(const float4*)(x + (long)min(p + RP_PL * j, q.nparts - 1) * q.stride);
+#pragma unroll
+        for (int j = 0; j < 7; ++j) {
+          if (p + RP_PL * j < q.nparts) {
+            a[0] += v[j].x; a[1] += v[j].y; a[2] += v[j].z; a[3] += v[j].w;
+          }
+        }
+      }
+    }
+#pragma unroll
+    for (int k = 0; k < 4; ++k) red[py][cx * 4 + k] = a[k];
+  } else {
+#pragma unroll
+    for (int k = 0; k < 4; ++k) {
+      const int c = c0 + cx + 16 * k;
+      if (c < q.n) {
+        int p = py;
+        for (; p + 7 * RP_PL < q.nparts; p += 8 * RP_PL) {
+          float v[8];
+#pragma unroll
+          for (int j = 0; j < 8; ++j) v[j] = q.part[(long)(p + RP_PL * j) * q.stride + c];
+#pragma unroll
+          for (int j = 0; j < 8; ++j) a[k] += v[j];
+        }
+        for (; p < q.nparts; p += RP_PL) a[k] += q.part[(long)p * q.stride + c];
+      }
+      red[py][cx + 16 * k] = a[k];
+    }
+  }
   __syncthreads();
-  if (py == 0 && c < q.n) {
+  const int c = c0 + threadIdx.x;
+  if (threadIdx.x < RP_CW && c < q.n) {
     double t = 0.0;
 #pragma unroll
-    for (int l = 0; l < RP_PL; ++l) t += red[l][cx];
-    q.out[c] = q.accumulate ? q.out[c] + (float)t : (float)t;
+    for (int l = 0; l < RP_PL; ++l) t += red[l][threadIdx.x];
+    const long o = q.tr_rows > 0 && c < q.tr_rows * q.tr_cols ? (long)(c % q.tr_rows) * q.tr_cols + c / q.tr_rows : c;
+    q.out[o] = q.accumulate ? q.out[o] + (float)t : (float)t;
   }
 }
 
@@ -186,10 +224,13 @@
   int rc = 0;
   for (int i = 0; i < n; ++i) {
     const ea_reduce_prob& e = probs[i];
-    if (!(e.part && e.out && e.n > 0 && e.nparts >= 0 && e.stride >= e.n)) { rc = EA_ERR_BAD_ARG; break; }
+    const bool tr_ok = e.tr_rows == 0 ? e.tr_cols == 0
+                                      : e.tr_rows > 0 && e.tr_cols > 0 && (long)e.tr_rows * e.tr_cols <= e.n;
+    if (!(e.part && e.out && e.n > 0 && e.nparts >= 0 && e.stride >= e.n && tr_ok)) { rc = EA_ERR_BAD_ARG; break; }
     ReduceProbD& d = host[i];
     d.part = e.part; d.out = e.out; d.stride = e.stride;
     d.nparts = e.nparts; d.n = e.n; d.accumulate = e.accumulate;
+    d.tr_rows = e.tr_rows; d.tr_cols = e.tr_cols;
     d.item0 = (int)items;
     items += ea_cdiv(e.n, RP_CW);
   }
diff --git a/espnet-1_amd/espnet_amd/deferred.py b/espnet-1_amd/espnet_amd/deferred.py
--- a/espnet-1_amd/espnet_amd/deferred.py
+++ b/espnet-1_amd/espnet_amd/deferred.py
@@ -123,9 +123,9 @@
         self._account(x)
         return True
 
-    def add_reduce(self, part, nparts, n, stride, out, accumulate=True):
+    def add_reduce(self, part, nparts, n, stride, out, accumulate=True, tr=(0, 0)):
         self._claim(out, n)
-        self.reduces.append((part, nparts, n, stride, out, accumulate))
+        self.reduces.append((part, nparts, n, stride, out, accumulate, 0, tr))
         self._account(part)
 
     def tensors(self):
@@ -150,16 +150,15 @@
             off = 0
             for i, ((x, rows, n, ld, out, acc), rpp, nrb) in enumerate(zip(colsums, rpps, nrbs)):
                 arr[i] = ColsumProb(x.data_ptr(), part.data_ptr() + 4 * off, ld, rows, n, dt(x), rpp)
-                reduces.append((part, nrb, n, n, out, acc, off))
+                reduces.append((part, nrb, n, n, out, acc, off, (0, 0)))
                 off += nrb * n
             lib.ea_grouped_table_bytes(len(colsums), ctypes.addressof(cb), ctypes.addressof(rb))
             ws = scratch("colsum", cb.value, dev)
             lib.ea_colsum_grouped(len(colsums), ctypes.addressof(arr), ws.data_ptr(), ws.numel(), stream())
         arr = (ReduceProb * len(reduces))()
         for i, r in enumerate(reduces):
-            part, nparts, n, stride, out, acc = r[:6]
-            off = r[6] if len(r) > 6 else 0
-            arr[i] = ReduceProb(part.data_ptr() + 4 * off, out.data_ptr(), stride, nparts, n, int(acc))
+            part, nparts, n, stride, out, acc, off, tr = r
+            arr[i] = ReduceProb(part.data_ptr() + 4 * off, out.data_ptr(), stride, nparts, n, int(acc), *tr)
         lib.ea_grouped_table_bytes(len(reduces), ctypes.addressof(cb), ctypes.addressof(rb))
         ws = scratch("reduce", rb.value, dev)
         lib.ea_reduce_grouped(len(reduces), ctypes.addressof(arr), ws.data_ptr(), ws.numel(), stream())
diff --git a/espnet-1_amd/espnet_amd/hip_ops.py b/espnet-1_amd/espnet_amd/hip_ops.py
--- a/espnet-1_amd/espnet_amd/hip_ops.py
+++ b/espnet-1_amd/espnet_amd/hip_ops.py
@@ -9,7 +9,7 @@
 import torch
 
 from . import deferred, streams
-from ._lib import ACT_NONE, EPI_STORE, Epilogue, HipError, dt, lib
+from ._lib import ACT_NONE, EPI_DACT, EPI_STORE, Epilogue, HipError, dt, lib
 from .deferred import (REDUCE_Q, WGRAD_Q, deferred_tensors, deferred_wgrad, flush_deferred,
                        flush_wgrad_side, fork_event, grad_ready, join_wgrad, wgrad)
 from .streams import aux, join_aux, mark_aux_fork, on_side, scratch, stream, take_aux_fork
@@ -262,16 +262,38 @@
     return ts.get(w)
 
 
-def linear_dx(dy, w, out, *, epi: Epilogue = None):
+EPI_COLSUM = os.environ.get("EA_EPI_COLSUM", "1") != "0"
+
+
+def linear_dx(dy, w, out, *, epi: Epilogue = None, colsum_out=None):
     M, N, lda = _rows(dy)
     K = w.shape[1]
     _, _, ldc = _rows(out)
+    part = None
+    if colsum_out is not None and EPI_COLSUM and epi is not None and epi.kind == EPI_DACT and M > 0:
+        part = torch.empty((M + 63) // 64, K, dtype=torch.float32, device=out.device)
+        epi.colsum_part = part.data_ptr()
+        epi.ldpart = K
     wt = _transposed(w)
     if wt is not None:
-        return gemm(dy, wt, out, M=M, N=K, K=N, a_kmajor=1, b_kmajor=1, lda=lda, ldb=wt.stride(0),
-                    ldc=ldc, epi=epi)
-    return gemm(dy, w, out, M=M, N=K, K=N, a_kmajor=1, b_kmajor=0, lda=lda, ldb=w.stride(0),
-                ldc=ldc, epi=epi)
+        gemm(dy, wt, out, M=M, N=K, K=N, a_kmajor=1, b_kmajor=1, lda=lda, ldb=wt.stride(0), ldc=ldc, epi=epi)
+    else:
+        gemm(dy, w, out, M=M, N=K, K=N, a_kmajor=1, b_kmajor=0, lda=lda, ldb=w.stride(0), ldc=ldc, epi=epi)
+    if colsum_out is None:
+        return out
+    n = colsum_out.numel()
+    if K % n:
+        raise HipError("colsum_out must divide the output width")
+    nrows = ctypes.c_int(0)
+    if part is not None:
+        epi.colsum_part = None
+        lib.ea_gemm_colsum_rows(ctypes.addressof(nrows))
+    if nrows.value:
+        reduce_rows(part, nrows.value * (K // n), n, n, colsum_out)
+    else:
+        with wgrad(out):
+            colsum(out if n == K else out.reshape(-1, n), colsum_out)
+    return out
 
 
 def linear_dw(dy, x, dw, *, accumulate=False, post=None):
@@ -357,6 +379,38 @@
     lib.ea_reduce_partials(nparts, n, part.data_ptr(), stride, out.data_ptr(), int(accumulate), stream())
 
 
+DEFER_DWCONV = os.environ.get("EA_DEFER_DWCONV", "1") != "0"
+
+
+def dwconv_bwd(B, T, C, K, x, w, dy, dx, dw, dbias, *, g2=None, dg2=None):
+    rowlen = C * (K + 1)
+    glu = g2 is not None
+    if REDUCE_Q.active and DEFER_DWCONV and K in (3, 5, 7, 15, 31):
+        np_ = ctypes.c_int(0)
+        lib.ea_dwconv_stats_parts(B, T, ctypes.addressof(np_))
+        part = torch.empty(np_.value * rowlen, dtype=torch.float32, device=dy.device)
+        if glu:
+            lib.ea_dwconv_glu_bwd_partials(B, T, C, K, ptr(x), w.data_ptr(), dy.data_ptr(), g2.data_ptr(),
+                                           dg2.data_ptr(), part.data_ptr(), part.numel(), ctypes.addressof(np_),
+                                           stream())
+        else:
+            lib.ea_dwconv_bwd_partials(B, T, C, K, x.data_ptr(), w.data_ptr(), dy.data_ptr(), dx.data_ptr(),
+                                       part.data_ptr(), part.numel(), ctypes.addressof(np_), stream())
+        if dbias.data_ptr() == dw.data_ptr() + 4 * C * K:
+            REDUCE_Q.add_reduce(part, np_.value, rowlen, rowlen, dw, True, tr=(C, K))
+        else:
+            REDUCE_Q.add_reduce(part, np_.value, C * K, rowlen, dw, True, tr=(C, K))
+            REDUCE_Q.add_reduce(part[C * K:], np_.value, C, rowlen, dbias, True)
+        return
+    ws, wn = f32_ws(dy.device, B * ((T + 31) // 32) * rowlen + 1024)
+    if glu:
+        lib.ea_dwconv_glu_bwd(B, T, C, K, ptr(x), w.data_ptr(), dy.data_ptr(), g2.data_ptr(), dg2.data_ptr(),
+                              dw.data_ptr(), dbias.data_ptr(), 1, ws, wn, stream())
+    else:
+        lib.ea_dwconv_bwd(B, T, C, K, x.data_ptr(), w.data_ptr(), dy.data_ptr(), dx.data_ptr(), dw.data_ptr(),
+                          dbias.data_ptr(), 1, ws, wn, stream())
+
+
 def colsum(x, out, accumulate=True, defer=True):
     rows, n, ld = _rows(x)
     if defer and REDUCE_Q.active and REDUCE_Q.add_colsum(x, rows, n, ld, out, accumulate):
diff --git a/espnet-1_amd/espnet_amd/layers/conformer.py b/espnet-1_amd/espnet_amd/layers/conformer.py
--- a/espnet-1_amd/espnet_amd/layers/conformer.py
+++ b/espnet-1_amd/espnet_amd/layers/conformer.py
@@ -142,10 +142,9 @@
     with ops.wgrad(dv, a):
         ops.linear_dw(dv, a, b.g(pre + ".w_2.weight"), accumulate=True)
     dh = empty(*h.shape, dtype=cd, device=dx.device)
-    ops.linear_dx(dv, b.w(pre + ".w_2.weight"), dh,
+    ops.linear_dx(dv, b.w(pre + ".w_2.weight"), dh, colsum_out=b.g(pre + ".w_1.bias"),
                   epi=ops.make_epi(EPI_DACT, act=ACT_SWISH, aux=h, drop_p=p, seed=seed_in))
     with ops.wgrad(dh, xn):
-        ops.colsum(dh, b.g(pre + ".w_1.bias"))
         ops.linear_dw(dh, xn, b.g(pre + ".w_1.weight"), accumulate=True)
     dxn = empty(N, d, dtype=cd, device=dx.device)
     ops.linear_dx(dh, b.w(pre + ".w_1.weight"), dxn)
@@ -310,20 +309,15 @@
         dg2 = empty(N, 2 * d, dtype=cd, device=dev)
         fuse = FUSE_DW_GLU and K in (3, 5, 7, 15, 31) and g2.dtype == torch.bfloat16
         if fuse:
-            w, wn = ops.f32_ws(dev, B * ((T + 31) // 32) * d * (K + 1) + 1024)
-            lib.ea_dwconv_glu_bwd(B, T, d, K, ops.ptr(glu), b.f(C + "depthwise_conv.weight").data_ptr(),
-                                  dy.data_ptr(), g2.data_ptr(), dg2.data_ptr(),
-                                  b.g(C + "depthwise_conv.weight").data_ptr(),
-                                  b.g(C + "depthwise_conv.bias").data_ptr(), 1, w, wn, ops.stream())
+            ops.dwconv_bwd(B, T, d, K, glu, b.f(C + "depthwise_conv.weight"), dy, None,
+                           b.g(C + "depthwise_conv.weight"), b.g(C + "depthwise_conv.bias"), g2=g2, dg2=dg2)
         else:
             if glu is None:
                 glu = empty(N, d, device=dev)
                 lib.ea_glu_fwd(N, d, g2.data_ptr(), ops.dt(g2), glu.data_ptr(), 0, ops.stream())
             dglu = empty(N, d, device=dev)
-            w, wn = ops.f32_ws(dev, B * ((T + 31) // 32) * d * (K + 1) + 1024)
-            lib.ea_dwconv_bwd(B, T, d, K, glu.data_ptr(), b.f(C + "depthwise_conv.weight").data_ptr(),
-                              dy.data_ptr(), dglu.data_ptr(), b.g(C + "depthwise_conv.weight").data_ptr(),
-                              b.g(C + "depthwise_conv.bias").data_ptr(), 1, w, wn, ops.stream())
+            ops.dwconv_bwd(B, T, d, K, glu, b.f(C + "depthwise_conv.weight"), dy, dglu,
+                           b.g(C + "depthwise_conv.weight"), b.g(C + "depthwise_conv.bias"))
             lib.ea_glu_bwd(N, d, g2.data_ptr(), ops.dt(g2), dglu.data_ptr(), dg2.data_ptr(), ops.stream())
         with ops.wgrad(dg2, xn3):
             ops.colsum(dg2, b.g(C + "pointwise_conv1.bias"))
diff --git a/espnet-1_amd/espnet_amd/layers/decoder.py b/espnet-1_amd/espnet_amd/layers/decoder.py
--- a/espnet-1_amd/espnet_amd/layers/decoder.py
+++ b/espnet-1_amd/espnet_amd/layers/decoder.py
@@ -223,12 +223,11 @@
                 ops.linear_dw(dv, a, b.g(ff + "w_2.weight"), accumulate=True)
             fork = ops.fork_event() if l < nb - 1 else None
             dh = empty(*h.shape, dtype=cd, device=dev)
-            ops.linear_dx(dv, b.w(ff + "w_2.weight"), dh,
+            ops.linear_dx(dv, b.w(ff + "w_2.weight"), dh, colsum_out=b.g(ff + "w_1.bias"),
                           epi=ops.make_epi(EPI_DACT, act=ACT_RELU, aux=h, drop_p=p, seed=sd(l, 5)))
             if fork is not None:
                 ops.flush_wgrad_side(after=fork)
             with ops.wgrad(dh, xn3):
-                ops.colsum(dh, b.g(ff + "w_1.bias"))
                 ops.linear_dw(dh, xn3, b.g(ff + "w_1.weight"), accumulate=True)
             dxn = empty(N, d, dtype=cd, device=dev)
             ops.linear_dx(dh, b.w(ff + "w_1.weight"), dxn)
diff --git a/espnet-1_amd/espnet_amd/layers/subsampling.py b/espnet-1_amd/espnet_amd/layers/subsampling.py
--- a/espnet-1_amd/espnet_amd/layers/subsampling.py
+++ b/espnet-1_amd/espnet_amd/layers/subsampling.py
@@ -236,10 +236,10 @@
         K2 = rup(P2, 64)
         dx2 = empty(P2 + 128, C, dtype=cd, device=dev)
         dx2[P2:].zero_()
-        ops.linear_dx(dv, wl, dx2[:P2].view(B * T2, F2 * C), epi=ops.make_epi(EPI_DACT, act=ACT_RELU, aux=x2r))
+        ops.linear_dx(dv, wl, dx2[:P2].view(B * T2, F2 * C), colsum_out=b.g("conv.2.bias"),
+                      epi=ops.make_epi(EPI_DACT, act=ACT_RELU, aux=x2r))
         ws_side = None
         with ops.wgrad(dx2, x1p, launches=True):
-            ops.colsum(dx2[:P2], b.g("conv.2.bias"))
             dw2 = empty(C, 9 * C, device=dev)
             geo, _, _, _ = phase_geo(B, T1, F1, T2, F2, C, CONV_WGRAD, zero=P1 * C)
             epi = ops.make_epi()
@@ -329,10 +329,9 @@
             ops.linear_dw(dv, x2r, dwl, accumulate=False,
                           post=lambda: ops.permute3(dwl, gw, C, F2, C, accumulate=True))
         dx2 = empty(B * T2, F2 * C, dtype=cd, device=dev)
-        ops.linear_dx(dv, wl, dx2, epi=ops.make_epi(EPI_DACT, act=ACT_RELU, aux=x2r))
+        ops.linear_dx(dv, wl, dx2, colsum_out=b.g("conv.2.bias"), epi=ops.make_epi(EPI_DACT, act=ACT_RELU, aux=x2r))
         dx2 = dx2.view(-1, C)
         with ops.wgrad(dx2, col2):
-            ops.colsum(dx2, b.g("conv.2.bias"))
             dw2 = empty(C, 9 * C, device=dev)
             g2 = b.g("conv.2.weight")
             ops.linear_dw(dx2, col2, dw2, accumulate=False,
diff --git a/espnet-1_amd/espnet_amd/layers/transformer.py b/espnet-1_amd/espnet_amd/layers/transformer.py
--- a/espnet-1_amd/espnet_amd/layers/transformer.py
+++ b/espnet-1_amd/espnet_amd/layers/transformer.py
@@ -102,10 +102,9 @@
         with ops.wgrad(dv, a):
             ops.linear_dw(dv, a, b.g("feed_forward.w_2.weight"), accumulate=True)
         dh = empty(*h.shape, dtype=cd, device=dev)
-        ops.linear_dx(dv, b.w("feed_forward.w_2.weight"), dh,
+        ops.linear_dx(dv, b.w("feed_forward.w_2.weight"), dh, colsum_out=b.g("feed_forward.w_1.bias"),
                       epi=ops.make_epi(EPI_DACT, act=ACT_RELU, aux=h, drop_p=p_ff, seed=sd(3)))
         with ops.wgrad(dh, xn2):
-            ops.colsum(dh, b.g("feed_forward.w_1.bias"))
             ops.linear_dw(dh, xn2, b.g("feed_forward.w_1.weight"), accumulate=True)
         dxn = empty(N, d, dtype=cd, device=dev)
         ops.linear_dx(dh, b.w("feed_forward.w_1.weight"), dxn)
diff --git a/include/espnet_amd.h b/include/espnet_amd.h
--- a/include/espnet_amd.h
+++ b/include/espnet_amd.h
@@ -24,6 +24,8 @@
   long ldaux;
   const float* resid;
   long ldr;
+  float* colsum_part;
+  long ldpart;
 } ea_epilogue;
 
 int ea_gemm(int dtype, int a_kmajor, int b_kmajor, int M, int N, int K,
@@ -32,7 +34,7 @@
             int batch, int nh,
             void* C, int c_dtype, long ldc, long sCb, long sCh,
             const ea_epilogue* epi, float* workspace, long ws_elems, void* stream);
-
+int ea_gemm_colsum_rows(int* rows);
 
 enum { EA_CONV_FWD = 1, EA_CONV_DGRAD = 2, EA_CONV_WGRAD = 3 };
 typedef struct ea_conv_geo {
@@ -135,6 +137,7 @@
   float* out;
   long stride;
   int nparts, n, accumulate;
+  int tr_rows, tr_cols;
 } ea_reduce_prob;
 int ea_colsum_grouped(int n, const ea_colsum_prob* probs, void* ws, long ws_bytes, void* stream);
 int ea_reduce_grouped(int n, const ea_reduce_prob* probs, void* ws, long ws_bytes, void* stream);
@@ -216,6 +219,11 @@
 int ea_dwconv_glu_bwd(int B, int T, int C, int K, const float* x, const float* w, const float* dy,
                       const void* g2, void* dg2, float* dw, float* dbias, int accumulate_params,
                       float* workspace, long ws_elems, void* stream);
+int ea_dwconv_bwd_partials(int B, int T, int C, int K, const float* x, const float* w, const float* dy,
+                           float* dx, float* part, long part_elems, int* nparts, void* stream);
+int ea_dwconv_glu_bwd_partials(int B, int T, int C, int K, const float* x, const float* w, const float* dy,
+                               const void* g2, void* dg2, float* part, long part_elems, int* nparts,
+                               void* stream);
 int ea_dwconv_fwd_glu(int B, int T, int C, int K, const void* g2, const float* w, const float* bias,
                       float* y, void* stream);
 int ea_dwconv_fwd_glu_stats(int B, int T, int C, int K, const void* g2, const float* w, const float* bias,
```

Result: no change. 1930 utterances/s, median of 6 (+1.0%).
